# yuang-chen/of-spmm

Hardware: AMD Instinct MI355X
Metric: SpMM effective GFLOP/s + achieved HBM GB/s vs roofline, 1/2/4/8 MI355X (higher is better)
Workload: dtype f32; 1 GPU; products: CSR 2449029x2449029, 123718280 nnz x dense N=128; m=2449029, k=2449029, nnz=123718280, n=128, index=int32, parallelism=single GPU

## Files before the change

include/ofx_spmm.h:

```cpp
#ifndef OFX_SPMM_H_
#define OFX_SPMM_H_

#include <stddef.h>
#include <stdint.h>

#ifdef __cplusplus
extern "C" {
#endif

#define OFX_OK 0
#define OFX_EINVAL 1
#define OFX_EDEVICE 2
#define OFX_ENOMEM 3
#define OFX_EUNSUPPORTED 4
#define OFX_ECOMM 5
#define OFX_EWORKSPACE 6
#define OFX_EPLAN 7
#define OFX_EINTERNAL 8

#define OFX_DT_FLOAT 2
#define OFX_DT_DOUBLE 3
#define OFX_DT_INT32 5
#define OFX_DT_INT64 6
#define OFX_DT_FLOAT16 9
#define OFX_DT_BFLOAT16 11

const char* ofx_last_error(void);
const char* ofx_version(void);

int ofx_device_error_check(void);

#define OFX_DEBUG_PLAN_SPIN_LIMIT 1
#define OFX_DEBUG_THROW_IN_COMPUTE 2
#define OFX_DEBUG_EXCHANGE_STALL 3
int ofx_debug_set(int knob, int64_t value);

#define OFX_STRUCT_MAGIC 0x4F465831u

typedef struct ofx_spmm_options {
  uint32_t struct_size;
  uint32_t magic;
  int64_t split_threshold;
  int64_t chunk;
  int32_t ordered;
  int32_t variant;
  int64_t heavy_threshold;
  int32_t planned;
  int32_t reserved;
  int64_t range_nnz;
} ofx_spmm_options;
#define OFX_SPMM_OPTIONS_MIN_SIZE 48u
#define OFX_SPMM_OPTIONS_INIT \
  {(uint32_t)sizeof(ofx_spmm_options), OFX_STRUCT_MAGIC, 0, 0, 0, 0, 0, 0, 0, 0}

int64_t ofx_spmm_default_split(int64_t n);

int ofx_spmm_csr_workspace_size(int idx_dtype, int val_dtype, int64_t m, int64_t k, int64_t n,
                                int64_t nnz, const ofx_spmm_options* opts, size_t* bytes);

int ofx_spmm_csr(void* stream, int idx_dtype, int val_dtype, int64_t m, int64_t k, int64_t n,
                 int64_t nnz, const void* row_ptr, const void* col_idx, const void* values,
                 const void* b, int64_t ldb, void* c, int64_t ldc, int64_t row_begin,
                 int64_t row_end, void* workspace, size_t workspace_bytes,
                 const ofx_spmm_options* opts);

int ofx_spmm_csr_gathered(void* stream, int idx_dtype, int val_dtype, int64_t m, int64_t k,
                          int64_t n, int64_t nnz, const void* row_ptr, const void* col_idx,
                          const void* values, const void* values_perm, const void* b,
                          int64_t ldb, void* c, int64_t ldc, int64_t row_begin, int64_t row_end,
                          void* workspace, size_t workspace_bytes, const ofx_spmm_options* opts);

int ofx_spmm_csr_plan(void* stream, int idx_dtype, int val_dtype, int64_t m, int64_t k, int64_t n,
                      int64_t nnz, const void* row_ptr, int64_t row_begin, int64_t row_end,
                      void* workspace, size_t workspace_bytes, const ofx_spmm_options* opts);

int ofx_spmm_csr_describe(int idx_dtype, int val_dtype, int64_t m, int64_t k, int64_t n,
                          int64_t nnz, const void* b, int64_t ldb, const void* c, int64_t ldc,
                          int64_t row_begin, int64_t row_end, const ofx_spmm_options* opts,
                          char* buf, size_t buf_bytes);

int ofx_debug_bounds_read(uint64_t* out, int reset);

#define OFX_ACT_NONE 0
#define OFX_ACT_RELU 1
int ofx_spmm_csr_fused(void* stream, int idx_dtype, int val_dtype, int64_t m, int64_t k, int64_t n,
                       int64_t nnz, const void* row_ptr, const void* col_idx, const void* values,
                       const void* b, int64_t ldb, void* c, int64_t ldc, int64_t row_begin,
                       int64_t row_end, const void* bias, int activation, void* workspace,
                       size_t workspace_bytes, const ofx_spmm_options* opts);
int ofx_spmm_csr_fused_cpu(int num_threads, int idx_dtype, int val_dtype, int64_t m, int64_t k,
                           int64_t n, int64_t nnz, const void* row_ptr, const void* col_idx,
                           const void* values, const void* b, int64_t ldb, void* c, int64_t ldc,
                           int64_t row_begin, int64_t row_end, const void* bias, int activation,
                           const ofx_spmm_options* opts);

int ofx_csr_validate(void* stream, int idx_dtype, int64_t m, int64_t k, int64_t nnz,
                     const void* row_ptr, const void* col_idx, void* flag_dev);

int ofx_spmm_csr_cpu(int num_threads, int idx_dtype, int val_dtype, int64_t m, int64_t k,
                     int64_t n, int64_t nnz, const void* row_ptr, const void* col_idx,
                     const void* values, const void* b, int64_t ldb, void* c, int64_t ldc,
                     int64_t row_begin, int64_t row_end, const ofx_spmm_options* opts);

int ofx_csr_transpose_workspace_size(int idx_dtype, int64_t m, int64_t k, int64_t nnz,
                                     size_t* bytes);
int ofx_csr_transpose(void* stream, int idx_dtype, int64_t m, int64_t k, int64_t nnz,
                      const void* row_ptr, const void* col_idx, void* out_row_ptr,
// ... 151 lines not shown
                       void* d_bias, int relu, void* workspace, size_t workspace_bytes);
int ofx_relu_bias_grad_cpu(int num_threads, int val_dtype, int64_t m, int64_t n, const void* y,
                           int64_t ldy, const void* dy, int64_t lddy, void* dx, int64_t lddx,
                           void* d_bias, int relu);

int ofx_balanced_range(int64_t total, int64_t parts, int64_t idx, int64_t* begin, int64_t* end);
int ofx_csr_row_slice(void* stream, int idx_dtype, const void* row_ptr, int64_t row_begin,
                      int64_t row_end, void* out_row_ptr);
int ofx_csr_row_slice_host(int idx_dtype, const void* row_ptr, int64_t row_begin,
                           int64_t row_end, void* out_row_ptr, int64_t* nnz_begin,
                           int64_t* nnz_end);

int ofx_device_count(int* count);
int ofx_set_device(int device);
int ofx_get_device(int* device);
int ofx_device_synchronize(void);
int ofx_malloc(void** ptr, size_t bytes);
int ofx_free(void* ptr);
int ofx_host_malloc(void** ptr, size_t bytes);
int ofx_host_free(void* ptr);
int ofx_stream_create(void** stream);
int ofx_stream_destroy(void* stream);
int ofx_stream_sync(void* stream);
#define OFX_MEMCPY_H2D 1
#define OFX_MEMCPY_D2H 2
#define OFX_MEMCPY_D2D 3
#define OFX_MEMCPY_DEFAULT 4
int ofx_memcpy_async(void* stream, void* dst, const void* src, size_t bytes, int kind);
int ofx_memset_async(void* stream, void* dst, int value, size_t bytes);
int ofx_event_create(void** event, int timing);
int ofx_event_destroy(void* event);
int ofx_event_record(void* event, void* stream);
int ofx_event_sync(void* event);
int ofx_event_elapsed_ms(void* start, void* end, float* ms);
int ofx_stream_wait_event(void* stream, void* event);
int ofx_graph_exec_create(void** exec);
int ofx_graph_exec_destroy(void* exec);
int ofx_graph_exec_stats(void* exec, int* instantiated, int64_t* instantiations, int64_t* updates,
                         int64_t* launches);
int ofx_stream_begin_capture(void* stream);
int ofx_stream_is_capturing(void* stream, int* capturing);
int ofx_stream_end_capture(void* stream, void* exec);
int ofx_graph_launch(void* exec, void* stream);

#define OFX_UNIQUE_ID_BYTES 128
int ofx_comm_get_unique_id(void* uid_out );
int ofx_comm_init_rank(void** comm, int nranks, const void* uid, int rank);
int ofx_comm_init_rank_deadline(void** comm, int nranks, const void* uid, int rank,
                                double timeout_s);
int ofx_comm_set_timeouts(void* comm, double call_timeout_s, double device_timeout_s);
int ofx_comm_abort(void* comm);
int ofx_comm_destroy(void* comm);
int ofx_comm_count(void* comm, int* nranks, int* rank);
int ofx_allgather(void* stream, const void* in, void* out, size_t count, int dtype, void* comm);
int ofx_allgather_p2p(void* stream, void* buf, size_t count, int dtype, void* comm);
#define OFX_PEER_HANDLE_BYTES 96
#define OFX_PEER_MAX_RANKS 16
int ofx_peer_export(const void* ptr, void* handle_out);
int ofx_peer_open(const void* handle, void** ptr_out);
int ofx_peer_close(void* ptr);
int ofx_peer_publish(void* stream);
int ofx_peer_pull(void* stream, int nranks, int rank, const void* const* peer_bufs, void* buf,
                  uint64_t slot_bytes);
int ofx_peer_pull_host(int nranks, int rank, const void* const* peer_bufs, void* buf,
                       uint64_t slot_bytes);
int ofx_allgather_pull(void* stream, void* comm, const void* const* peer_bufs, void* buf,
// ... 45 lines not shown
                                  const ofx_tensor_desc* values, int64_t a_num_rows,
                                  int64_t a_num_cols, const ofx_tensor_desc* b,
                                  ofx_tensor_desc* out);
int ofx_functional_spmm_csr_tmp_size(const ofx_tensor_desc* row_ptr,
                                     const ofx_tensor_desc* col_idx,
                                     const ofx_tensor_desc* values, int64_t a_num_rows,
                                     int64_t a_num_cols, const ofx_tensor_desc* b,
                                     size_t* bytes);
int ofx_functional_spmm_csr(void* stream, const ofx_tensor_desc* row_ptr,
                            const ofx_tensor_desc* col_idx, const ofx_tensor_desc* values,
                            int64_t a_num_rows, int64_t a_num_cols, const ofx_tensor_desc* b,
                            ofx_tensor_desc* out, void* tmp, size_t tmp_bytes);
int ofx_functional_spmm_csr_global(void* stream, const ofx_tensor_desc* row_ptr,
                                   const ofx_tensor_desc* col_idx, const ofx_tensor_desc* values,
                                   int64_t a_num_rows, int64_t a_num_cols, const ofx_tensor_desc* b,
                                   int64_t b_logical_cols, ofx_tensor_desc* out, void* tmp,
                                   size_t tmp_bytes, int hierarchy_ndim, const int64_t* hierarchy,
                                   const int32_t* out_split_axes, int64_t parallel_id,
                                   int num_threads, size_t* tmp_size_out);
typedef struct ofx_spmm_attrs {
  uint32_t struct_size;
  uint32_t magic;
  int64_t static_csr;
} ofx_spmm_attrs;
#define OFX_SPMM_ATTRS_MIN_SIZE 16u
#define OFX_SPMM_ATTRS_INIT {(uint32_t)sizeof(ofx_spmm_attrs), OFX_STRUCT_MAGIC, 0}
int ofx_functional_spmm_csr_global_attrs(
    void* stream, const ofx_tensor_desc* row_ptr, const ofx_tensor_desc* col_idx,
    const ofx_tensor_desc* values, int64_t a_num_rows, int64_t a_num_cols,
    const ofx_tensor_desc* b, int64_t b_logical_cols, ofx_tensor_desc* out, void* tmp,
    size_t tmp_bytes, int hierarchy_ndim, const int64_t* hierarchy, const int32_t* out_split_axes,
    int64_t parallel_id, int num_threads, size_t* tmp_size_out, const ofx_spmm_attrs* attrs);
int ofx_spmm_static_plans(int64_t* entries, int64_t* plans, int64_t* hits, int release);

int ofx_functional_spmm_csr_ex(void* stream, const ofx_tensor_desc* row_ptr,
                               const ofx_tensor_desc* col_idx, const ofx_tensor_desc* values,
                               int64_t a_num_rows, int64_t a_num_cols, const ofx_tensor_desc* b,
                               ofx_tensor_desc* out, void* tmp, size_t tmp_bytes,
                               int64_t parallel_id, int64_t parallel_num, int out_split_axis,
                               int num_threads);
int ofx_functional_fused_spmm_csr(void* stream, const ofx_tensor_desc* row_ptr,
                                  const ofx_tensor_desc* col_idx, const ofx_tensor_desc* values,
                                  const ofx_tensor_desc* b, const ofx_tensor_desc* bias,
                                  int64_t a_num_rows, int64_t a_num_cols, int relu,
                                  ofx_tensor_desc* out, void* tmp, size_t tmp_bytes,
                                  size_t* tmp_size_out);
int ofx_functional_fused_spmm_csr_attrs(void* stream, const ofx_tensor_desc* row_ptr,
                                        const ofx_tensor_desc* col_idx,
                                        const ofx_tensor_desc* values, const ofx_tensor_desc* b,
                                        const ofx_tensor_desc* bias, int64_t a_num_rows,
                                        int64_t a_num_cols, int relu, ofx_tensor_desc* out,
                                        void* tmp, size_t tmp_bytes, size_t* tmp_size_out,
                                        const ofx_spmm_attrs* attrs);
int ofx_functional_sddmm_csr(void* stream, const ofx_tensor_desc* row_ptr,
                             const ofx_tensor_desc* col_idx, const ofx_tensor_desc* a,
                             const ofx_tensor_desc* b, int64_t a_num_rows, int64_t a_num_cols,
                             ofx_tensor_desc* out, void* tmp, size_t tmp_bytes,
                             size_t* tmp_size_out);
int ofx_functional_sddmm_csr_attrs(void* stream, const ofx_tensor_desc* row_ptr,
                                   const ofx_tensor_desc* col_idx, const ofx_tensor_desc* a,
                                   const ofx_tensor_desc* b, int64_t a_num_rows,
                                   int64_t a_num_cols, ofx_tensor_desc* out, void* tmp,
                                   size_t tmp_bytes, size_t* tmp_size_out,
                                   const ofx_spmm_attrs* attrs);
int ofx_functional_csr_transpose(void* stream, const ofx_tensor_desc* row_ptr,
                                 const ofx_tensor_desc* col_idx, int64_t a_num_rows,
// ... 118 lines not shown
```

of-spmm_amd/csrc/device_shim.cpp:

```cpp
#include <hip/hip_runtime.h>

#include <atomic>
#include <cstring>
#include <mutex>

#include "ofx_internal.h"

namespace {
constexpr int kErrWords = 16;
std::atomic<unsigned*> g_err_words{nullptr};
unsigned* g_err_dev = nullptr;
std::once_flag g_err_once;
}

namespace ofx {
unsigned* device_error_words() {
  std::call_once(g_err_once, [] {
    int count = 0;
    if (hipGetDeviceCount(&count) != hipSuccess || count <= 0) {
      (void)hipGetLastError();
      return;
    }
    hipStreamCaptureMode mode = hipStreamCaptureModeRelaxed;
    (void)hipThreadExchangeStreamCaptureMode(&mode);
// ... 64 lines not shown
extern "C" int ofx_device_synchronize(void) {
  return ::ofx::guarded(__func__, [&]() -> int {
    OFX_HIP_CHECK(hipDeviceSynchronize());
    OFX_TAKE_DEVICE_ERROR("device_synchronize");
    return OFX_OK;
  });
}
extern "C" int ofx_malloc(void** ptr, size_t bytes) {
  return ::ofx::guarded(__func__, [&]() -> int {
    OFX_REQUIRE(ptr, OFX_EINVAL, "malloc: NULL");
    *ptr = nullptr;
    if (bytes == 0) return OFX_OK;
    hipError_t e = hipMalloc(ptr, (bytes + 511) / 512 * 512);
    if (e != hipSuccess) {
      (void)hipGetLastError();
      return ofx::fail(OFX_ENOMEM, "hipMalloc(%zu) failed: %s", bytes, hipGetErrorString(e));
    }
    return OFX_OK;
  });
}
extern "C" int ofx_free(void* ptr) {
  return ::ofx::guarded(__func__, [&]() -> int {
    if (ptr) OFX_HIP_CHECK(hipFree(ptr));
    return OFX_OK;
  });
}
extern "C" int ofx_host_malloc(void** ptr, size_t bytes) {
  return ::ofx::guarded(__func__, [&]() -> int {
    OFX_REQUIRE(ptr, OFX_EINVAL, "host_malloc: NULL");
    OFX_HIP_CHECK(hipHostMalloc(ptr, bytes ? bytes : 1, hipHostMallocDefault));
    return OFX_OK;
  });
}
extern "C" int ofx_host_free(void* ptr) {
  return ::ofx::guarded(__func__, [&]() -> int {
    if (ptr) OFX_HIP_CHECK(hipHostFree(ptr));
    return OFX_OK;
  });
}
extern "C" int ofx_stream_create(void** stream) {
  return ::ofx::guarded(__func__, [&]() -> int {
    OFX_REQUIRE(stream, OFX_EINVAL, "stream_create: NULL");
    hipStream_t s;
    OFX_HIP_CHECK(hipStreamCreateWithFlags(&s, hipStreamNonBlocking));
    *stream = s;
    return OFX_OK;
  });
}
extern "C" int ofx_stream_destroy(void* stream) {
  return ::ofx::guarded(__func__, [&]() -> int {
    if (stream) OFX_HIP_CHECK(hipStreamDestroy(static_cast<hipStream_t>(stream)));
    return OFX_OK;
  });
}
extern "C" int ofx_stream_sync(void* stream) {
  return ::ofx::guarded(__func__, [&]() -> int {
    OFX_HIP_CHECK(hipStreamSynchronize(static_cast<hipStream_t>(stream)));
    OFX_TAKE_DEVICE_ERROR("stream_sync");
    return OFX_OK;
  });
}
extern "C" int ofx_memcpy_async(void* stream, void* dst, const void* src, size_t bytes, int kind) {
  return ::ofx::guarded(__func__, [&]() -> int {
    if (bytes == 0) return OFX_OK;
    hipMemcpyKind k;
    switch (kind) {
// ... 9 lines not shown
}
extern "C" int ofx_memset_async(void* stream, void* dst, int value, size_t bytes) {
  return ::ofx::guarded(__func__, [&]() -> int {
    if (bytes == 0) return OFX_OK;
    OFX_HIP_CHECK(hipMemsetAsync(dst, value, bytes, static_cast<hipStream_t>(stream)));
    return OFX_OK;
  });
}
extern "C" int ofx_event_create(void** event, int timing) {
  return ::ofx::guarded(__func__, [&]() -> int {
    OFX_REQUIRE(event, OFX_EINVAL, "event_create: NULL");
    hipEvent_t e;
    OFX_HIP_CHECK(hipEventCreateWithFlags(&e, timing ? hipEventDefault : hipEventDisableTiming));
    *event = e;
    return OFX_OK;
  });
}
extern "C" int ofx_event_destroy(void* event) {
  return ::ofx::guarded(__func__, [&]() -> int {
    if (event) OFX_HIP_CHECK(hipEventDestroy(static_cast<hipEvent_t>(event)));
    return OFX_OK;
  });
}
extern "C" int ofx_event_record(void* event, void* stream) {
  return ::ofx::guarded(__func__, [&]() -> int {
    OFX_HIP_CHECK(hipEventRecord(static_cast<hipEvent_t>(event), static_cast<hipStream_t>(stream)));
    return OFX_OK;
  });
}
extern "C" int ofx_event_sync(void* event) {
  return ::ofx::guarded(__func__, [&]() -> int {
    OFX_HIP_CHECK(hipEventSynchronize(static_cast<hipEvent_t>(event)));
    OFX_TAKE_DEVICE_ERROR("event_sync");
    return OFX_OK;
  });
}
extern "C" int ofx_event_elapsed_ms(void* start, void* end, float* ms) {
  return ::ofx::guarded(__func__, [&]() -> int {
    OFX_REQUIRE(ms, OFX_EINVAL, "event_elapsed_ms: NULL");
    OFX_HIP_CHECK(hipEventElapsedTime(ms, static_cast<hipEvent_t>(start),
                                      static_cast<hipEvent_t>(end)));
    return OFX_OK;
  });
}
extern "C" int ofx_stream_wait_event(void* stream, void* event) {
  return ::ofx::guarded(__func__, [&]() -> int {
    OFX_HIP_CHECK(hipStreamWaitEvent(static_cast<hipStream_t>(stream),
                                     static_cast<hipEvent_t>(event), 0));
    return OFX_OK;
  });
}

namespace {
struct GraphExec {
  hipGraphExec_t exec = nullptr;
  int device = -1;
  int64_t instantiations = 0;
  int64_t updates = 0;
  int64_t launches = 0;
};
}

extern "C" int ofx_graph_exec_create(void** exec) {
  return ::ofx::guarded(__func__, [&]() -> int {
    OFX_REQUIRE(exec, OFX_EINVAL, "graph_exec_create: NULL");
    *exec = new GraphExec();
// ... 109 lines not shown
```

of-spmm_amd/csrc/spmm_common.h:

```cpp
#ifndef OFX_SPMM_COMMON_H_
#define OFX_SPMM_COMMON_H_

#include <stdint.h>
#include <string.h>

#include "ofx_spmm.h"

#if defined(__HIPCC__) || defined(__HIP__)
#include <hip/hip_runtime.h>
#define OFX_HD __host__ __device__ __forceinline__
#else
#define OFX_HD static inline
#endif

namespace ofx {

struct bf16 {
  uint16_t x;
};
struct f16 {
  uint16_t x;
};

OFX_HD float bits_to_f32(uint32_t u) { return __builtin_bit_cast(float, u); }
// ... 89 lines not shown
  if (idx_dtype == OFX_DT_INT32) return f((int32_t*)nullptr);
  return f((int64_t*)nullptr);
}
template <typename F>
int by_types(int idx_dtype, int val_dtype, F&& f) {
  return by_index(idx_dtype, [&](auto* ip) -> int {
    switch (val_dtype) {
      case OFX_DT_FLOAT: return f((float*)nullptr, ip);
      case OFX_DT_DOUBLE: return f((double*)nullptr, ip);
      case OFX_DT_BFLOAT16: return f((bf16*)nullptr, ip);
      default: return f((f16*)nullptr, ip);
    }
  });
}

OFX_HD int64_t default_split(int64_t n) {
  int64_t t = n > 0 ? (int64_t)65536 / n : 512;
  if (t < 128) t = 128;
  if (t > 512) t = 512;
  int64_t p = 128;
  while (p * 2 <= t) p *= 2;
  return p;
}

struct Schedule {
  int64_t split;
  int64_t chunk;
  int64_t heavy;
  int32_t variant;
  int32_t planned;
  int32_t force_bin;
};

static inline Schedule resolve_schedule(int64_t n, const ofx_spmm_options* o) {
  Schedule s;
  s.variant = o ? o->variant : 0;
  s.planned = o ? o->planned : 0;
  s.force_bin = 0;
  const int64_t h = o ? o->heavy_threshold : 0;
  s.heavy = h > 0 ? h : (h < 0 ? INT64_MAX : 0);
  if (o && o->ordered) {
    s.split = INT64_MAX;
    s.chunk = INT64_MAX;
    return s;
  }
  s.split = (o && o->split_threshold > 0) ? o->split_threshold : default_split(n);
  s.chunk = (o && o->chunk > 0) ? o->chunk : s.split;
  if (s.chunk > s.split) s.chunk = s.split;
  return s;
}

OFX_HD int64_t auto_heavy(int64_t nrows, int64_t nnz) {
  const int64_t mean = nrows > 0 ? (nnz + nrows - 1) / nrows : 1;
  return 5 * mean < 16 ? 16 : 5 * mean;
}

OFX_HD int64_t num_chunks(int64_t len, int64_t chunk) { return len / chunk; }

OFX_HD uint64_t splitmix64(uint64_t x) {
  x += 0x9e3779b97f4a7c15ull;
  x = (x ^ (x >> 30)) * 0xbf58476d1ce4e5b9ull;
  x = (x ^ (x >> 27)) * 0x94d049bb133111ebull;
  return x ^ (x >> 31);
}
OFX_HD uint64_t hash2(uint64_t seed, uint64_t i) { return splitmix64(splitmix64(seed) ^ i); }
OFX_HD float u_pm1(uint64_t h) { return float((int64_t)(h >> 40) - (1 << 23)) * (1.0f / (1 << 23)); }
// ... 10 lines not shown
```

of-spmm_amd/csrc/spmm_csr.hip:

```cpp
#pragma clang fp contract(off)

#include <hip/hip_runtime.h>

#include <algorithm>
#include <climits>
#include <type_traits>

#include "ofx_internal.h"
#include "spmm_common.h"
#include "spmm_plan.h"
#include "spmm_launch.h"
#include "dbg_bounds.h"

namespace ofx {
namespace {

using plan::ws_layout;

template <typename I>
__global__ void csr_validate_kernel(const I* __restrict__ rp, const I* __restrict__ col,
                                    int64_t m, int64_t k, int64_t nnz, unsigned int* flag) {
  const int64_t stride = (int64_t)gridDim.x * blockDim.x;
  const int64_t t0 = (int64_t)blockIdx.x * blockDim.x + threadIdx.x;
  for (int64_t i = t0; i <= m; i += stride) {
// ... 132 lines not shown
    OFX_READ_OPTIONS(opts, "spmm_csr_describe");
    int rc = check_common(idx_dtype, val_dtype, m, k, n, nnz);
    if (rc) return rc;
    OFX_REQUIRE(0 <= row_begin && row_begin < row_end && row_end <= m && n > 0, OFX_EINVAL,
                "spmm_csr_describe: empty launch (rows [%lld, %lld), n=%lld)", (long long)row_begin,
                (long long)row_end, (long long)n);
    OFX_REQUIRE(ldb >= n && ldc >= n, OFX_EINVAL, "spmm_csr_describe: ldb / ldc < n");
    const int64_t nrows = row_end - row_begin;
    const int64_t nnz_est = launch_nnz(m, nrows, nnz, opts);
    Launch L{nullptr, nullptr, nullptr, nullptr, b, const_cast<void*>(c), ldb, ldc, row_begin, nrows,
             n, nnz, launch_schedule(nrows, nnz_est, n, resolve_schedule(n, opts)), nullptr, 0,
             nullptr, OFX_ACT_NONE, k, nullptr, nnz_est, buf, buf_bytes};
    if (idx_dtype == OFX_DT_INT32) return launch_idx<int32_t>(val_dtype, L);
    return launch_idx<int64_t>(val_dtype, L);
  });
}

extern "C" int ofx_spmm_csr_gathered(void* stream, int idx_dtype, int val_dtype, int64_t m,
                                     int64_t k, int64_t n, int64_t nnz, const void* row_ptr,
                                     const void* col_idx, const void* values,
                                     const void* values_perm, const void* b, int64_t ldb, void* c,
                                     int64_t ldc, int64_t row_begin, int64_t row_end,
                                     void* workspace, size_t workspace_bytes,
                                     const ofx_spmm_options* opts) {
  return ::ofx::guarded(__func__, [&]() -> int {
    OFX_REQUIRE(nnz == 0 || values_perm != nullptr, OFX_EINVAL,
                "spmm_csr_gathered: NULL values_perm with nnz=%lld", (long long)nnz);
    return spmm_entry(stream, idx_dtype, val_dtype, m, k, n, nnz, row_ptr, col_idx, values,
                      values_perm, b, ldb, c, ldc, row_begin, row_end, nullptr, OFX_ACT_NONE,
                      workspace, workspace_bytes, opts);
  });
}

extern "C" int ofx_spmm_csr_plan(void* stream, int idx_dtype, int val_dtype, int64_t m,
                                 int64_t k, int64_t n, int64_t nnz, const void* row_ptr,
                                 int64_t row_begin, int64_t row_end, void* workspace,
                                 size_t workspace_bytes, const ofx_spmm_options* opts) {
  return ::ofx::guarded(__func__, [&]() -> int {
    OFX_TAKE_DEVICE_ERROR("spmm_csr_plan");
    OFX_READ_OPTIONS(opts, "spmm_csr_plan");
    int rc = check_common(idx_dtype, val_dtype, m, k, n, nnz);
    if (rc) return rc;
    OFX_REQUIRE(0 <= row_begin && row_begin <= row_end && row_end <= m, OFX_EINVAL,
                "spmm_csr_plan: row range [%lld, %lld) outside [0, %lld)", (long long)row_begin,
                (long long)row_end, (long long)m);
    const int64_t nrows = row_end - row_begin;
    if (nrows == 0 || n == 0) return OFX_OK;
    const int64_t nnz_est = launch_nnz(m, nrows, nnz, opts);
    const Schedule s = launch_schedule(nrows, nnz_est, n, resolve_schedule(n, opts));
    if (use_small_form(nrows, nnz_est, n, s)) return OFX_OK;
    const plan::WsLayout w = plan::ws_layout(nrows, nnz, n, acc_bytes_of(val_dtype), s);
    if (w.total == 0) return OFX_OK;
    OFX_REQUIRE(row_ptr != nullptr, OFX_EINVAL, "spmm_csr_plan: NULL row_ptr");
    OFX_REQUIRE(workspace != nullptr && workspace_bytes >= w.total, OFX_EWORKSPACE,
                "spmm_csr_plan: workspace of %zu bytes is smaller than the %zu bytes required",
                workspace_bytes, w.total);
    hipStream_t st = static_cast<hipStream_t>(stream);
  #ifdef OFX_DEBUG_BOUNDS
    {
      dbg::HostBounds hb;
      hb.add(row_ptr, (uint64_t)((row_end + 1) * (idx_dtype == OFX_DT_INT32 ? 4 : 8)));
      hb.add(workspace, workspace_bytes);
      OFX_REQUIRE(hb.publish(st, 3ull << 48) == 0, OFX_EDEVICE, "spmm_csr_plan: debug bounds");
    }
  #endif
    plan::WorkList wl{};
    char* ws = static_cast<char*>(workspace);
    if (idx_dtype == OFX_DT_INT32)
      return plan::launch_plan<int32_t>(st, static_cast<const int32_t*>(row_ptr), row_begin, nrows,
                                        nnz_est, s, w, ws, &wl);
    return plan::launch_plan<int64_t>(st, static_cast<const int64_t*>(row_ptr), row_begin, nrows,
                                      nnz_est, s, w, ws, &wl);
  });
}

extern "C" int ofx_spmm_csr_fused(void* stream, int idx_dtype, int val_dtype, int64_t m,
                                  int64_t k, int64_t n, int64_t nnz, const void* row_ptr,
                                  const void* col_idx, const void* values, const void* b,
                                  int64_t ldb, void* c, int64_t ldc, int64_t row_begin,
                                  int64_t row_end, const void* bias, int activation,
                                  void* workspace, size_t workspace_bytes,
                                  const ofx_spmm_options* opts) {
  return ::ofx::guarded(__func__, [&]() -> int {
    return spmm_entry(stream, idx_dtype, val_dtype, m, k, n, nnz, row_ptr, col_idx, values, nullptr,
                      b, ldb, c, ldc, row_begin, row_end, bias, activation, workspace,
                      workspace_bytes, opts);
  });
}

extern "C" int ofx_csr_validate(void* stream, int idx_dtype, int64_t m, int64_t k, int64_t nnz,
                                const void* row_ptr, const void* col_idx, void* flag_dev) {
  return ::ofx::guarded(__func__, [&]() -> int {
    OFX_REQUIRE(is_index_dtype(idx_dtype), OFX_EUNSUPPORTED, "csr_validate: bad index dtype %d",
                idx_dtype);
    OFX_REQUIRE(row_ptr && flag_dev && (nnz == 0 || col_idx), OFX_EINVAL,
                "csr_validate: NULL pointer");
    hipStream_t s = static_cast<hipStream_t>(stream);
    OFX_HIP_CHECK(hipMemsetAsync(flag_dev, 0, sizeof(unsigned int), s));
    int64_t work = std::max<int64_t>(m + 1, nnz);
    int64_t grid = std::min<int64_t>((work + 255) / 256, 4096);
    if (grid < 1) grid = 1;
    if (idx_dtype == OFX_DT_INT32)
      hipLaunchKernelGGL(csr_validate_kernel<int32_t>, dim3((unsigned)grid), dim3(256), 0, s,
                         static_cast<const int32_t*>(row_ptr), static_cast<const int32_t*>(col_idx),
                         m, k, nnz, static_cast<unsigned int*>(flag_dev));
// ... 98 lines not shown
```

of-spmm_amd/csrc/spmm_csr_impl.h:

```cpp
#ifndef OFX_SPMM_CSR_IMPL_H_
#define OFX_SPMM_CSR_IMPL_H_
#pragma clang fp contract(off)

#include <hip/hip_runtime.h>

#include <algorithm>
#include <climits>
#include <cstdio>
#include <cstring>
#include <type_traits>

#include "ofx_internal.h"
#include "spmm_common.h"
#include "spmm_plan.h"
#include "spmm_launch.h"
#include "dbg_bounds.h"

namespace ofx {
namespace {


using plan::WorkList;
using plan::WsLayout;
using plan::launch_plan;
// ... 479 lines not shown
        for (int e = 0; e < VEC; ++e) lds[i * W + gl * VEC + e] = Num<T>::mul(vv[u], Num<T>::load(bv[u].v[e]));
      }
    }
    __builtin_amdgcn_fence(__ATOMIC_RELEASE, "wavefront");
    __builtin_amdgcn_wave_barrier();
    __builtin_amdgcn_fence(__ATOMIC_ACQUIRE, "wavefront");
    if (q == 0) {
#pragma unroll 8
      for (int i = 0; i < cnt; ++i)
#pragma unroll
        for (int e = 0; e < VEC; ++e) acc[e] = acc[e] + lds[i * W + gl * VEC + e];
    }
    __builtin_amdgcn_wave_barrier();
  }
}

template <typename T, int VEC, bool NT>
__device__ __forceinline__ void store_row(T* __restrict__ p, const typename Num<T>::acc (&acc)[VEC],
                                          const T* __restrict__ bias, int act) {
  if (!OFX_DOK(p, sizeof(Pack<T, VEC>)) || (bias && !OFX_DOK(bias, sizeof(T) * VEC))) return;
  Pack<T, VEC> o;
  if (bias == nullptr && act == OFX_ACT_NONE) {
#pragma unroll
    for (int e = 0; e < VEC; ++e) o.v[e] = Num<T>::store(acc[e]);
  } else {
#pragma unroll
    for (int e = 0; e < VEC; ++e) o.v[e] = epilogue<T>(acc[e], bias, e, act);
  }
  if constexpr (NT && (sizeof(o) == 16 || sizeof(o) == 8 || sizeof(o) == 4 || sizeof(o) == 2)) {
    using R = typename RawVec<sizeof(o)>::type;
    __builtin_nontemporal_store(__builtin_bit_cast(R, o), reinterpret_cast<R*>(p));
  } else {
    *reinterpret_cast<Pack<T, VEC>*>(p) = o;
  }
}

template <typename A, int VEC, bool COH = false>
__device__ __forceinline__ void store_partial(A* __restrict__ p, const A (&acc)[VEC]) {
  if constexpr (COH) {
#pragma unroll
    for (int e = 0; e < VEC; ++e) coh_store(p + e, acc[e]);
  } else {
    if (!OFX_DOK(p, sizeof(A) * VEC)) return;
#pragma unroll
    for (int e = 0; e < VEC; ++e) p[e] = acc[e];
  }
}

template <typename T, int VEC, int L, bool SH>
__device__ __forceinline__ void hub_tail(unsigned* __restrict__ arrive, int64_t slot0, int64_t nc,
                                         const typename Num<T>::acc* __restrict__ part,
                                         T* __restrict__ C, int64_t ldc, int64_t lr, int64_t n,
                                         int gl, bool member, int lead_lane,
                                         const T* __restrict__ bias, int act) {
#pragma clang fp contract(off)
  using A = typename Num<T>::acc;
  wait_stores();
  unsigned old = 0;
  if (member && gl == 0)
    old = __hip_atomic_fetch_add(arrive + slot0, 1u, __ATOMIC_RELAXED, __HIP_MEMORY_SCOPE_AGENT);
  old = __shfl(old, lead_lane);
  if ((int64_t)old != nc - 1) return;
  if (!member) return;
  for (int64_t c0 = 0; c0 < n; c0 += (int64_t)L * VEC) {
    int64_t cc = c0 + (int64_t)gl * VEC;
    if (cc >= n) continue;
// ... 327 lines not shown
      if (chain && active)
        store_row<T, VEC, K::NT>(C + hr * ldc + cc, split_row ? total : acc,
                                 bias ? bias + cc : nullptr, act);
    }
  }
}

#ifdef OFX_AB_WPE
#define OFX_MAIN_WPE __attribute__((amdgpu_waves_per_eu(OFX_AB_WPE)))
#else
#define OFX_MAIN_WPE
#endif
template <typename T>
__device__ __attribute__((noinline)) void poison_output(T* __restrict__ C, int64_t ldc,
                                                        int64_t nrows, int64_t n) {
  const T p = poison_value<T>();
  const int64_t total = nrows * n;
  const int64_t stride = (int64_t)gridDim.x * blockDim.x;
  for (int64_t e = (int64_t)blockIdx.x * blockDim.x + threadIdx.x; e < total; e += stride)
    C[(e / n) * ldc + e % n] = p;
}

template <typename T, typename I, typename K>
__global__ void __launch_bounds__(64 * K::WPB) OFX_MAIN_WPE
    spmm_main_kernel(const I* __restrict__ rp, const I* __restrict__ col,
                     const T* __restrict__ val, const I* __restrict__ vperm,
                     const T* __restrict__ B, int64_t ldb, int64_t kb,
                     T* __restrict__ C, int64_t ldc, int64_t row_begin, int64_t nrows, int64_t n,
                     int64_t split, int64_t chunk, int64_t heavy,
                     const unsigned long long* __restrict__ counters,
                     const int64_t* __restrict__ items, const int64_t* __restrict__ order,
                     typename Num<T>::acc* __restrict__ part, const T* __restrict__ bias,
                     int act, int64_t wave_blocks, int64_t block_base,
                     unsigned* __restrict__ arrive, unsigned* err) {
  using A = typename Num<T>::acc;
  constexpr int VEC = K::VEC, LPR = K::LPR, kWaves = K::WPB;
  const int64_t bid = block_base + (int64_t)blockIdx.x;
  if (counters != nullptr && !plan::plan_valid(counters)) {
    if (bid == 0 && threadIdx.x == 0) plan::raise_device_error(err, plan::kErrPlanInvalid);
    poison_output<T>(C, ldc, nrows, n);
    return;
  }
  constexpr int GPW = 64 / LPR;
  const int lane = threadIdx.x & 63;
  const int wave = __builtin_amdgcn_readfirstlane(threadIdx.x >> 6);
  const int gl = lane & (LPR - 1);
  const int gbase = lane & ~(LPR - 1);
  const int gsub = LPR == 64 ? 0 : lane / LPR;
  if constexpr (K::WH && LPR < 64) {
    using KW = WaveMap<K>;
    constexpr int WV = KW::VEC, WL = KW::LPR;
    if (bid < wave_blocks) {
      const int wgl = lane & (WL - 1);
      const int64_t nchunks = (int64_t)OFX_LD(counters + 0);
      const int64_t nheavy = (int64_t)OFX_LD(counters + 3) - (int64_t)OFX_LD(counters + 2);
      for (int64_t w = bid * kWaves + wave; w < nchunks + nheavy; w += wave_blocks * kWaves) {
        int64_t wr, wc = -1;
        if (w < nchunks) {
          wr = OFX_LD(items + (2 * w + 0));
          wc = OFX_LD(items + (2 * w + 1));
        } else {
          wr = plan::order_row(order, nrows, nheavy, w - nchunks);
        }
        wr = uniform64(wr);
        wc = uniform64(wc);
        const int64_t rs = (int64_t)OFX_LD(rp + (row_begin + wr));
        const int64_t re = (int64_t)OFX_LD(rp + (row_begin + wr + 1));
        int64_t j0 = rs, j1 = re;
        if (wc >= 0) {
          j0 = rs + wc * chunk;
          j1 = (re - j0 - chunk < chunk) ? re : j0 + chunk;
        }
        for (int64_t c0 = 0; c0 < n; c0 += (int64_t)WL * WV) {
          int64_t cc = c0 + (int64_t)wgl * WV;
          const bool active = cc < n;
          if constexpr (K::SH && WV > 1) {
            if (active && cc + WV > n) cc = n - WV;
          }
          A acc[WV];
#pragma unroll
          for (int e = 0; e < WV; ++e) acc[e] = A(0);
          if constexpr (K::XL) {
            __shared__ A xl_lds[K::WPB][KW::XL_FLOATS];
            accumulate_wave_xl<T, I, KW>(col, val, vperm, brows<T, K::BUF>(B, c0, cc, active, ldb, kb),
                                         j0, j1, lane, wgl, xl_lds[wave], acc);
          } else {
            accumulate_wave<T, I, KW>(col, val, vperm, brows<T, K::BUF>(B, c0, cc, active, ldb, kb),
                                      j0, j1, lane, wgl, acc);
          }
          if (active && lane < WL) {
            if (wc >= 0)
              store_partial<A, WV, K::LR>(part + w * n + cc, acc);
            else
              store_row<T, WV, K::NT>(C + wr * ldc + cc, acc, bias ? bias + cc : nullptr, act);
          }
        }
        if constexpr (K::LR) {
          if (wc >= 0)
            hub_tail<T, WV, WL, K::SH && (WV > 1)>(arrive, w - wc, num_chunks(re - rs, chunk), part, C, ldc,
                                       wr, n, wgl, lane < WL, 0, bias, act);
        }
      }
      return;
    }
  }
  if constexpr (K::BI) {
    if (bid < wave_blocks) {
      __shared__ __attribute__((aligned(16))) SmallLds<T, I, K> lds;
      constexpr int W = SmallForm<T, I, K>::W;
      const int64_t w = bid;
      const int64_t nchunks = (int64_t)OFX_LD(counters + 0);
      const int64_t nheavy = (int64_t)OFX_LD(counters + 3) - (int64_t)OFX_LD(counters + 2);
      if (w >= nchunks + nheavy) return;
      int64_t wr, wc = -1;
      if (w < nchunks) {
        wr = OFX_LD(items + (2 * w + 0));
        wc = OFX_LD(items + (2 * w + 1));
      } else {
        wr = plan::order_row(order, nrows, nheavy, w - nchunks);
      }
      wr = uniform64(wr);
      wc = uniform64(wc);
      const int64_t rs = (int64_t)OFX_LD(rp + (row_begin + wr));
      const int64_t re = (int64_t)OFX_LD(rp + (row_begin + wr + 1));
      int64_t j0 = rs, j1 = re;
      if (wc >= 0) {
        j0 = rs + wc * chunk;
        j1 = (re - j0 - chunk < chunk) ? re : j0 + chunk;
      }
      const int gb = wave * GPW + gsub;
      const bool chain = wave == 0 && gsub == 0;
      for (int64_t c0 = 0; c0 < n; c0 += W) {
        const int64_t cc = c0 + (int64_t)gl * VEC;
        const bool active = cc < n;
        A acc[VEC];
#pragma unroll
        for (int e = 0; e < VEC; ++e) acc[e] = A(0);
        block_accumulate<T, I, K>(col, val, vperm, brows<T, K::BUF>(B, c0, cc, active, ldb, kb), j0, j1, gb, gl,
                                  chain, lds, acc);
        if (chain && active) {
          if (wc >= 0)
            store_partial<A, VEC, K::LR>(part + w * n + cc, acc);
          else
            store_row<T, VEC, K::NT>(C + wr * ldc + cc, acc, bias ? bias + cc : nullptr, act);
        }
      }
      if constexpr (K::LR) {
        if (wc >= 0 && chain)
          hub_tail<T, VEC, LPR, K::SH>(arrive, w - wc, num_chunks(re - rs, chunk), part, C, ldc, wr,
                                       n, gl, true, gbase, bias, act);
      }
      return;
    }
  }
  int64_t g = ((bid - ((K::WH || K::BI) ? wave_blocks : 0)) * kWaves + wave) * GPW +
              gsub;
  if constexpr ((K::WH && LPR < 64) || K::BI) {
    if (order != nullptr)
      g += (int64_t)OFX_LD(counters + 0) + (int64_t)OFX_LD(counters + 3) -
           (int64_t)OFX_LD(counters + 2);
  }
  constexpr int64_t kIdxExcluded = 16;
#if defined(OFX_LIGHT_ORDER)
  constexpr bool kIdx = false;
#else
  constexpr bool kIdx = true;
#endif
  int64_t lr, c = -1;
  bool by_index = false;
  if (order == nullptr) {
    if (g >= nrows) return;
    lr = g;
  } else {
    const int64_t nchunks = (int64_t)OFX_LD(counters + 0);
    const int64_t nhubs = (int64_t)OFX_LD(counters + 1);
    const int64_t nheavy = (int64_t)OFX_LD(counters + 3) - (int64_t)OFX_LD(counters + 2);
#if defined(OFX_LIGHT_INDEX)
    const bool idx = true;
#else
    const bool idx = kIdx && (nhubs + nheavy) * kIdxExcluded <= nrows;
#endif
    if (g < nchunks) {
      lr = OFX_LD(items + (2 * g + 0));
      c = OFX_LD(items + (2 * g + 1));
    } else if (g < nchunks + nheavy || !idx) {
      const int64_t q = g - nchunks;
      if (q >= nrows - nhubs) return;
      lr = plan::order_row(order, nrows, nheavy, q);
    } else {
      lr = g - nchunks - nheavy;
      if (lr >= nrows) return;
      by_index = true;
    }
  }
  if constexpr (LPR == 64) {
    lr = uniform64(lr);
    c = uniform64(c);
  }
  const int64_t rs = (int64_t)OFX_LD(rp + (row_begin + lr));
  const int64_t re = (int64_t)OFX_LD(rp + (row_begin + lr + 1));
  if (by_index && (re - rs > split || re - rs > heavy)) return;
  int64_t j0 = rs, j1 = re;
  if (c >= 0) {
    j0 = rs + c * chunk;
    j1 = (re - j0 - chunk < chunk) ? re : j0 + chunk;
  }
  for (int64_t c0 = 0; c0 < n; c0 += (int64_t)LPR * VEC) {
    int64_t cc = c0 + (int64_t)gl * VEC;
    const bool active = cc < n;
    if constexpr (K::SH) {
      if (active && cc + VEC > n) cc = n - VEC;
    }
    A acc[VEC];
#pragma unroll
    for (int e = 0; e < VEC; ++e) acc[e] = A(0);
    accumulate<T, I, K>(col, val, vperm, brows<T, K::BUF>(B, c0, cc, active, ldb, kb), j0, j1, gl, gbase, active,
                        acc);
    if (active) {
      if (c >= 0)
        store_partial<A, VEC, K::LR>(part + g * n + cc, acc);
      else
        store_row<T, VEC, K::NT>(C + lr * ldc + cc, acc, bias ? bias + cc : nullptr, act);
    }
  }
  if constexpr (K::LR) {
    if (c >= 0)
      hub_tail<T, VEC, LPR, K::SH>(arrive, g - c, num_chunks(re - rs, chunk), part, C, ldc, lr, n,
                                   gl, true, gbase, bias, act);
  }
}


template <typename T, int VEC, int L>
__global__ void __launch_bounds__(kBlock)
    spmm_reduce_kernel(const unsigned long long* __restrict__ counters,
                       const int64_t* __restrict__ hubs,
                       const typename Num<T>::acc* __restrict__ part, T* __restrict__ C,
                       int64_t ldc, int64_t n, const T* __restrict__ bias, int act) {
#pragma clang fp contract(off)
  using A = typename Num<T>::acc;
  using P = Pack<A, VEC>;
  constexpr int kPre = 16;
  if (!plan::plan_valid(counters)) return;
  const int64_t nhubs = (int64_t)OFX_LD(counters + 1);
  const int gl = threadIdx.x % L;
  const int64_t groups = (int64_t)gridDim.x * (kBlock / L);
  for (int64_t h = (int64_t)blockIdx.x * (kBlock / L) + threadIdx.x / L; h < nhubs; h += groups) {
    const int64_t lr = OFX_LD(hubs + (3 * h + 0));
    const int64_t slot = OFX_LD(hubs + (3 * h + 1));
    const int64_t nc = OFX_LD(hubs + (3 * h + 2));
    for (int64_t c = (int64_t)gl * VEC; c < n; c += (int64_t)L * VEC) {
      const A* p = part + slot * n + c;
      A acc[VEC];
#pragma unroll
      for (int e = 0; e < VEC; ++e) acc[e] = A(0);
      int64_t q = 0;
      for (; q + kPre <= nc; q += kPre) {
        P v[kPre];
#pragma unroll
        for (int u = 0; u < kPre; ++u) v[u] = OFX_LD(reinterpret_cast<const P*>(p + (q + u) * n));
#pragma unroll
        for (int u = 0; u < kPre; ++u) {
#pragma unroll
          for (int e = 0; e < VEC; ++e) acc[e] = acc[e] + v[u].v[e];
        }
      }
      for (; q < nc; ++q) {
        const P v = OFX_LD(reinterpret_cast<const P*>(p + q * n));
#pragma unroll
        for (int e = 0; e < VEC; ++e) acc[e] = acc[e] + v.v[e];
      }
      if (bias && !OFX_DOK(bias + c, sizeof(T) * VEC)) continue;
#pragma unroll
      for (int e = 0; e < VEC; ++e) OFX_ST(&C[lr * ldc + c + e], epilogue<T>(acc[e], bias, c + e, act));
    }
  }
}

template <typename T, int VEC>
int launch_reduce_vec(hipStream_t s, int64_t max_hubs, int64_t n,
                      const unsigned long long* counters, const int64_t* hubs,
                      const typename Num<T>::acc* part, T* C, int64_t ldc, const T* bias, int act) {
  const int64_t lanes = (n + VEC - 1) / VEC;
  int l = 4;
  while (l < 64 && l < lanes) l *= 2;
  const int64_t per_block = kBlock / l;
  int64_t grid = (max_hubs + per_block - 1) / per_block;
  if (grid > kMaxReduceBlocks) grid = kMaxReduceBlocks;
#define OFX_REDUCE(LL)                                                                        \
  hipLaunchKernelGGL((spmm_reduce_kernel<T, VEC, LL>), dim3((unsigned)grid), dim3(kBlock), 0, s, \
                     counters, hubs, part, C, ldc, n, bias, act)
  switch (l) {
    case 4: OFX_REDUCE(4); break;
    case 8: OFX_REDUCE(8); break;
    case 16: OFX_REDUCE(16); break;
    case 32: OFX_REDUCE(32); break;
    default: OFX_REDUCE(64); break;
  }
#undef OFX_REDUCE
  OFX_HIP_CHECK(hipGetLastError());
  return OFX_OK;
}

template <typename T>
int launch_reduce(hipStream_t s, int64_t max_hubs, int64_t n, const unsigned long long* counters,
                  const int64_t* hubs, const typename Num<T>::acc* part, T* C, int64_t ldc,
                  const T* bias, int act) {
  using A = typename Num<T>::acc;
  constexpr int kVec = 16 / (int)sizeof(A);
  if ((n * (int64_t)sizeof(A)) % 16 == 0)
    return launch_reduce_vec<T, kVec>(s, max_hubs, n, counters, hubs, part, C, ldc, bias, act);
  return launch_reduce_vec<T, 1>(s, max_hubs, n, counters, hubs, part, C, ldc, bias, act);
}

int pick_vec(int elem_bytes, const Launch& L, int forced_vec, int cap = 16) {
  const int maxvec = std::min(16 / elem_bytes, cap);
  for (int v = maxvec; v >= 1; v /= 2) {
    if (forced_vec && v != forced_vec) continue;
    const size_t vb = (size_t)v * elem_bytes;
    if (L.n % v == 0 && L.ldb % v == 0 && L.ldc % v == 0 &&
        ((uintptr_t)L.b % vb) == 0 && ((uintptr_t)L.c % vb) == 0)
      return v;
  }
  return 0;
}

int pick_lpr(int64_t n, int vec) {
  const int64_t lanes = (n + vec - 1) / vec;
  int l = 4;
  while (l < 64 && l < lanes) l *= 2;
  return l;
}

template <typename T, typename I, typename K>
int describe_cfg(const Launch& L, const char* kind) {
  const char* form = std::strcmp(kind, "small") == 0 ? "small"
                     : K::BI                         ? "mid"
                     : (K::WH && K::HL > 0)          ? "narrow"
                     : K::PF                         ? "prefetch"
                                                     : "bandwidth";
  const size_t ws = std::strcmp(kind, "small") == 0
                        ? 0
                        : ws_layout(L.nrows, L.nnz, L.n, sizeof(typename Num<T>::acc), L.sched).total;
  std::snprintf(L.describe, L.describe_bytes,
                "form=%s kernel=%s VEC=%d LPR=%d U=%d WPB=%d NT=%d PF=%d WH=%d BI=%d BUF=%d SH=%d "
// ... 21 lines not shown
  void* zero = nullptr;
  OFX_HIP_CHECK(hipGetSymbolAddress(&zero, HIP_SYMBOL(g_zero_row)));
  hb.add(zero, kZeroRowBytes);
  const unsigned long long flags = (unsigned long long)K::NT | (unsigned long long)K::PF << 1 |
                                   (unsigned long long)K::BNT << 2 | (unsigned long long)K::WH << 3 |
                                   (unsigned long long)K::BI << 4 | (unsigned long long)K::BUF << 5 |
                                   (unsigned long long)K::SH << 6 | (unsigned long long)K::LR << 7;
  const unsigned long long tag = (unsigned long long)K::VEC | (unsigned long long)K::LPR << 8 |
                                 (unsigned long long)K::U << 16 | flags << 24 |
                                 (unsigned long long)K::HL << 32 | (unsigned long long)K::HU << 40 |
                                 kind << 48;
  OFX_REQUIRE(hb.publish(L.stream, tag) == 0, OFX_EDEVICE, "spmm_csr: debug bounds not published");
  return OFX_OK;
}
#endif

template <typename T, typename I, typename K>
int launch_cfg(const Launch& L) {
  if (L.describe != nullptr) return describe_cfg<T, I, K>(L, "main");
  using A = typename Num<T>::acc;
  constexpr int GPW = 64 / K::LPR;
  constexpr int64_t GPB = (int64_t)K::WPB * GPW;
  const I* rp = static_cast<const I*>(L.rp);
  const I* col = static_cast<const I*>(L.col);
  const T* val = static_cast<const T*>(L.val);
  const T* B = static_cast<const T*>(L.b);
  T* C = static_cast<T*>(L.c);
  const WsLayout w = ws_layout(L.nrows, L.nnz, L.n, sizeof(A), L.sched);
  const bool plan = w.total > 0;
#ifdef OFX_DEBUG_BOUNDS
  if (const int rc = debug_publish<T, I, K>(L, 1)) return rc;
#endif
  WorkList wl{};
  if (plan) {
    OFX_REQUIRE(L.ws != nullptr && L.ws_bytes >= w.total, OFX_EWORKSPACE,
                "spmm_csr: workspace of %zu bytes is smaller than the %zu bytes required",
                L.ws_bytes, w.total);
    if (L.sched.planned) {
      plan::worklist_of(w, static_cast<char*>(L.ws), &wl);
    } else {
      const int rc = launch_plan<I>(L.stream, rp, L.row_begin, L.nrows, L.nnz_est, L.sched, w,
                                    static_cast<char*>(L.ws), &wl);
      if (rc) return rc;
    }
  }
  unsigned long long* counters = wl.counters;
  int64_t *hub = wl.hubs, *items = wl.items, *order = wl.order;
  A* part = reinterpret_cast<A*>(wl.part);
  const int64_t heavy = L.sched.heavy == 0 ? auto_heavy(L.nrows, L.nnz_est) : L.sched.heavy;
  const int64_t heavy_bound =
      heavy == INT64_MAX ? 0 : std::min<int64_t>(L.nrows, L.nnz / (heavy + 1) + 1);
  const int64_t bi_items = w.max_chunks + heavy_bound;
  constexpr int64_t kWaveItemBlocks = 2048;
  const bool wh = K::WH && K::LPR < 64 && plan;
  const int64_t wave_blocks = wh ? std::min<int64_t>((bi_items + K::WPB - 1) / K::WPB, kWaveItemBlocks)
                              : (K::BI && plan) ? bi_items
                                                : 0;
  const int64_t work = L.nrows + (plan && !wh && !K::BI ? bi_items : 0);
  const int64_t grid = wave_blocks + (work + GPB - 1) / GPB;
  constexpr int64_t kLaunchBlocks = ((int64_t)1 << 31) / (64 * K::WPB);
  for (int64_t b0 = 0; b0 < grid; b0 += kLaunchBlocks) {
    const int64_t nb = std::min(kLaunchBlocks, grid - b0);
    hipLaunchKernelGGL((spmm_main_kernel<T, I, K>), dim3((unsigned)nb), dim3(64 * K::WPB), 0,
                       L.stream, rp, col, val, static_cast<const I*>(L.vperm), B, L.ldb, L.b_rows,
                       C, L.ldc, L.row_begin, L.nrows, L.n, plan ? L.sched.split : INT64_MAX,
                       plan ? L.sched.chunk : INT64_MAX, heavy, counters, items, order, part,
                       static_cast<const T*>(L.bias), L.act, wave_blocks, b0, wl.arrive,
                       plan ? device_error_words() : nullptr);
    OFX_HIP_CHECK(hipGetLastError());
  }
  if (plan && w.max_hubs > 0 && !K::LR)
    return launch_reduce<T>(L.stream, w.max_hubs, L.n, counters, hub, part, C, L.ldc,
                            static_cast<const T*>(L.bias), L.act);
  return OFX_OK;
}


template <typename T, typename I, typename K>
int launch_small(const Launch& L) {
  if (L.describe != nullptr) return describe_cfg<T, I, K>(L, "small");
  using SF = SmallForm<T, I, K>;
  const int64_t light =
      (L.sched.heavy > 0 && L.sched.heavy != INT64_MAX) ? L.sched.heavy : (int64_t)kSmallLight * K::U;
  const int64_t grid = (L.nrows + SF::RPB - 1) / SF::RPB;
#ifdef OFX_DEBUG_BOUNDS
  if (const int rc = debug_publish<T, I, K>(L, 2)) return rc;
#endif
  OFX_REQUIRE(grid < (int64_t)UINT32_MAX, OFX_EINVAL, "spmm_csr: too many rows (%lld)",
              (long long)L.nrows);
  hipLaunchKernelGGL((spmm_small_kernel<T, I, K>), dim3((unsigned)grid), dim3(64 * K::WPB), 0,
                     L.stream, static_cast<const I*>(L.rp), static_cast<const I*>(L.col),
                     static_cast<const T*>(L.val), static_cast<const I*>(L.vperm),
                     static_cast<const T*>(L.b), L.ldb, L.b_rows, static_cast<T*>(L.c), L.ldc,
                     L.row_begin,
                     L.nrows, L.n, L.sched.split, L.sched.chunk, light,
                     static_cast<const T*>(L.bias), L.act);
  OFX_HIP_CHECK(hipGetLastError());
  return OFX_OK;
}

template <typename T, typename I, typename K>
int launch_small_or_planned(const Launch& L) {
  if (use_small_form(L.nrows, L.nnz_est, L.n, L.sched)) return launch_small<T, I, K>(L);
  return launch_cfg<T, I, K>(L);
}

// ... 262 lines not shown
```

of-spmm_amd/csrc/spmm_plan.h:

```cpp
#ifndef OFX_SPMM_PLAN_H_
#define OFX_SPMM_PLAN_H_

#include <hip/hip_runtime.h>

#include <atomic>
#include <chrono>
#include <climits>

#include "ofx_internal.h"
#include "spmm_common.h"
#include "dbg_bounds.h"

namespace ofx {

template <typename A>
__device__ __forceinline__ A coh_load(const A* p) {
  if (!OFX_DOK(p, sizeof(A))) return A(0);
#ifdef OFX_AB_UNORDERED_HANDOFF
  return *(volatile const A*)p;
#else
  return __hip_atomic_load(const_cast<A*>(p), __ATOMIC_RELAXED, __HIP_MEMORY_SCOPE_AGENT);
#endif
}
template <typename A>
// ... 11 lines not shown
namespace {

constexpr int kBlock = 256;

inline size_t align_up(size_t x, size_t a) { return (x + a - 1) / a * a; }

constexpr int64_t kPlanRptRows = int64_t(1) << 18;
inline int plan_rpt(int64_t nrows) { return nrows <= kPlanRptRows ? 4 : 16; }
constexpr int kBins = 2;
constexpr int kPlanVals = 2 + kBins;
constexpr int64_t kOwnItems = 8;
constexpr int kLookWords = 16;
constexpr int kLookWin = 4;
constexpr unsigned long long kAgg = 1, kInc = 2;
constexpr int kEpoch = 4, kHostTag = 5, kOk = 6, kFail = 7, kPoison = 8, kCounterWords = 9;
constexpr int kSpinLimit = 1 << 22;

__host__ __device__ __forceinline__ unsigned long long plan_tag(unsigned long long epoch,
                                                               unsigned long long host_tag) {
  return (splitmix64(epoch * 0x9e3779b97f4a7c15ull + splitmix64(host_tag)) >> 2) | 1ull;
}

__device__ __forceinline__ bool plan_valid(const unsigned long long* __restrict__ counters) {
  const unsigned long long e = OFX_LDP(counters + kEpoch), h = OFX_LDP(counters + kHostTag);
  const unsigned long long ok = OFX_LDP(counters + kOk), fl = OFX_LDP(counters + kFail);
  const unsigned long long poison = OFX_LDP(counters + kPoison);
  return ok != 0 && ok == plan_tag(e - 1, h) && fl != ok && poison != ok;
}

constexpr int kErrPlanFailed = 0, kErrPlanInvalid = 1;
__device__ __forceinline__ void raise_device_error(unsigned* err, int which) {
  if (err != nullptr)
    __hip_atomic_store(err + which, 1u, __ATOMIC_RELAXED, __HIP_MEMORY_SCOPE_SYSTEM);
}

template <typename I>
__device__ __forceinline__ int plan_row(const I* __restrict__ rp, int64_t row_begin, int64_t nrows,
                                        int64_t g, int64_t split, int64_t chunk, int64_t heavy,
                                        int64_t& nc) {
  nc = 0;
  if (g >= nrows) return -2;
  const int64_t len = (int64_t)OFX_LDP(rp + (row_begin + g + 1)) -
                      (int64_t)OFX_LDP(rp + (row_begin + g));
  if (len > split) {
    nc = num_chunks(len, chunk);
    return -1;
  }
  if (heavy == INT64_MAX) return kBins - 1;
  int64_t t = heavy;
  for (int b = 0; b < kBins - 1; ++b, t >>= 2)
    if (len > t) return b;
  return kBins - 1;
}

__device__ __forceinline__ int64_t order_row(const int64_t* __restrict__ order, int64_t nrows,
                                             int64_t nheavy, int64_t q) {
  return q < nheavy ? OFX_LDP(order + (nrows - 1 - q)) : OFX_LDP(order + (q - nheavy));
}

__device__ __forceinline__ void block_scan_vals(int64_t (&v)[kPlanVals], int64_t (&tot)[kPlanVals]) {
  constexpr int kWaves = kBlock / 64;
  __shared__ int64_t wsum[kPlanVals][kWaves];
  const int lane = threadIdx.x & 63, wv = threadIdx.x >> 6;
  int64_t inc[kPlanVals];
#pragma unroll
  for (int i = 0; i < kPlanVals; ++i) inc[i] = v[i];
// ... 85 lines not shown
#pragma unroll
  for (int q = 0; q < RPT; ++q) {
    unsigned long long big = __ballot(cls[q] == -1 && nc[q] > kOwnItems);
    while (big) {
      const int src = __ffsll((long long)big) - 1;
      big &= big - 1;
      const int64_t g = (int64_t)__shfl((long long)(base + q), src);
      const int64_t s0 = (int64_t)__shfl((long long)first[q], src);
      const int64_t ncs = (int64_t)__shfl((long long)nc[q], src);
      for (int64_t c = threadIdx.x & 63; c < ncs; c += 64) {
        OFX_STP(items + (2 * (s0 + c) + 0), g);
        OFX_STP(items + (2 * (s0 + c) + 1), c);
      }
    }
  }
}

__device__ __forceinline__ unsigned long long look_status(unsigned long long* look, int64_t b) {
  return coh_load(look + b * kLookWords);
}
__device__ __forceinline__ void look_publish(unsigned long long* look, int64_t b,
                                             unsigned long long status) {
  wait_stores();
  coh_store(look + b * kLookWords, status);
}

template <int RPT, typename I>
__global__ void __launch_bounds__(kBlock)
    spmm_plan_kernel(const I* __restrict__ rp, int64_t row_begin, int64_t nrows, int64_t split,
                     int64_t chunk, int64_t heavy, unsigned long long* __restrict__ look,
                     unsigned long long host_tag, int64_t nblocks,
                     unsigned long long* __restrict__ counters, int64_t* __restrict__ hubs,
                     int64_t* __restrict__ items, int64_t* __restrict__ order,
                     unsigned* __restrict__ arrive, int spin_limit, unsigned* err) {
  __shared__ int64_t s_off[kPlanVals];
  __shared__ int s_fail;
  int cls[RPT];
  int64_t nc[RPT], v[kPlanVals], tot[kPlanVals];
  const int64_t b = blockIdx.x;
  const int64_t base = (b * kBlock + (int64_t)threadIdx.x) * RPT;
  const unsigned long long dev_epoch = threadIdx.x < 64 ? coh_load(counters + kEpoch) : 0ull;
  plan_thread<RPT>(rp, row_begin, nrows, base, split, chunk, heavy, cls, nc, v);
  block_scan_vals(v, tot);
  if (threadIdx.x < 64) {
    const unsigned long long epoch = plan_tag(dev_epoch, host_tag);
    const int lane = threadIdx.x;
    unsigned long long* my = look + b * kLookWords;
    if (lane == 0) {
#pragma unroll
      for (int i = 0; i < kPlanVals; ++i) {
        coh_store(my + 1 + i, (unsigned long long)tot[i]);
        if (b == 0) coh_store(my + 1 + kPlanVals + i, (unsigned long long)tot[i]);
      }
      look_publish(look, b, epoch << 2 | (b == 0 ? kInc : kAgg));
    }
    int64_t pre[kPlanVals] = {};
    bool failed = spin_limit == 0 && b > 0;
    for (int64_t end = failed ? 0 : b; end > 0; end -= 64 * kLookWin) {
      int64_t p[kLookWin];
      unsigned long long st[kLookWin];
#pragma unroll
      for (int w = 0; w < kLookWin; ++w) {
        p[w] = end - 1 - 64 * w - lane;
        st[w] = 0;
      }
      for (int spins = 0;;) {
        bool waiting = false;
// ... 44 lines not shown
      s_fail = failed ? 1 : 0;
      if (b > 0 && !failed) {
#pragma unroll
        for (int i = 0; i < kPlanVals; ++i)
          coh_store(my + 1 + kPlanVals + i, (unsigned long long)(pre[i] + tot[i]));
        look_publish(look, b, epoch << 2 | kInc);
      }
#pragma unroll
      for (int i = 0; i < kPlanVals; ++i) s_off[i] = pre[i];
    }
    if (lane == 0 && failed) {
      coh_store(counters + kFail, epoch);
      coh_store(counters + kPoison, plan_tag(dev_epoch + 1, host_tag));
      raise_device_error(err, kErrPlanFailed);
    }
    if (lane == 0 && b == nblocks - 1) {
      if (!failed) {
        OFX_STP(counters + 0, (unsigned long long)(pre[1] + tot[1]));
        OFX_STP(counters + 1, (unsigned long long)(pre[0] + tot[0]));
        OFX_STP(counters + 2, 0ull);
        OFX_STP(counters + 3, (unsigned long long)(pre[2] + tot[2]));
        OFX_STP(counters + kHostTag, host_tag);
      }
      OFX_STP(counters + kOk, failed ? 0ull : epoch);
      OFX_STP(counters + kEpoch, dev_epoch + 1);
    }
  }
  __syncthreads();
  if (s_fail) return;
  int64_t off[kPlanVals];
#pragma unroll
  for (int i = 0; i < kPlanVals; ++i) off[i] = s_off[i];
  plan_write_rows(cls, nc, v, off, base, nrows, hubs, items, order, arrive);
}

struct WsLayout {
  size_t counters, look, hubs, items, order, arrive, part, total;
  int64_t max_hubs, max_chunks, plan_blocks;
};

constexpr int64_t kMinBinRows = 16384;

WsLayout ws_layout(int64_t nrows, int64_t nnz, int64_t n, size_t acc_bytes, const Schedule& s) {
  WsLayout w{};
  const bool bin = s.heavy != INT64_MAX && (nrows >= kMinBinRows || s.force_bin);
  const bool hub = s.split != INT64_MAX && nnz > s.split;
  if (!bin && !hub) return w;
  w.max_hubs = s.split == INT64_MAX ? 0 : nnz / (s.split + 1) + 1;
  w.max_chunks = s.split == INT64_MAX ? 0 : nnz / s.chunk + 1;
  const int64_t rows_per_block = (int64_t)kBlock * plan_rpt(nrows);
  w.plan_blocks = (nrows + rows_per_block - 1) / rows_per_block;
  const int64_t look_blocks = (nrows + (int64_t)kBlock * 4 - 1) / ((int64_t)kBlock * 4);
  size_t off = 0;
  w.counters = off;
  off = align_up(off + kCounterWords * sizeof(unsigned long long), 256);
  w.look = off;
  off = align_up(off + (size_t)look_blocks * kLookWords * sizeof(unsigned long long), 256);
  w.hubs = off;
  off = align_up(off + (size_t)w.max_hubs * 3 * sizeof(int64_t), 256);
  w.items = off;
  off = align_up(off + (size_t)w.max_chunks * 2 * sizeof(int64_t), 256);
  w.order = off;
  off = align_up(off + (size_t)nrows * sizeof(int64_t), 256);
  w.arrive = off;
  off = align_up(off + (size_t)w.max_chunks * sizeof(unsigned), 256);
  w.part = off;
  off = align_up(off + (size_t)w.max_chunks * (size_t)n * acc_bytes, 256);
  w.total = off;
  return w;
}

struct WorkList {
  unsigned long long* counters;
  int64_t* hubs;
  int64_t* items;
  int64_t* order;
  unsigned* arrive;
  void* part;
};

inline void worklist_of(const WsLayout& w, char* ws, WorkList* wl) {
  wl->counters = reinterpret_cast<unsigned long long*>(ws + w.counters);
  wl->hubs = reinterpret_cast<int64_t*>(ws + w.hubs);
  wl->items = reinterpret_cast<int64_t*>(ws + w.items);
  wl->order = reinterpret_cast<int64_t*>(ws + w.order);
  wl->arrive = reinterpret_cast<unsigned*>(ws + w.arrive);
  wl->part = ws + w.part;
}

inline unsigned long long next_host_tag() {
  static std::atomic<unsigned long long> counter{
      splitmix64((unsigned long long)std::chrono::steady_clock::now().time_since_epoch().count() ^
                 (unsigned long long)(uintptr_t)&counter)};
  return (splitmix64(counter.fetch_add(1)) >> 2) | 1ull;
}

template <typename I>
int launch_plan(hipStream_t stream, const I* rp, int64_t row_begin, int64_t nrows, int64_t nnz,
                const Schedule& sched, const WsLayout& w, char* ws, WorkList* wl) {
  const int64_t heavy = sched.heavy == 0 ? auto_heavy(nrows, nnz) : sched.heavy;
  worklist_of(w, ws, wl);
  auto* look = reinterpret_cast<unsigned long long*>(ws + w.look);
  OFX_REQUIRE(w.plan_blocks < (int64_t)UINT32_MAX, OFX_EINVAL, "spmm_csr: too many rows to plan");
  const unsigned long long host_tag = next_host_tag();
  const int spin = debug_knob(OFX_DEBUG_PLAN_SPIN_LIMIT, kSpinLimit);
  unsigned* err = device_error_words();
  if (plan_rpt(nrows) == 4)
    hipLaunchKernelGGL((spmm_plan_kernel<4, I>), dim3((unsigned)w.plan_blocks), dim3(kBlock), 0,
                       stream, rp, row_begin, nrows, sched.split, sched.chunk, heavy, look, host_tag,
                       w.plan_blocks, wl->counters, wl->hubs, wl->items, wl->order, wl->arrive,
                       spin, err);
  else
    hipLaunchKernelGGL((spmm_plan_kernel<16, I>), dim3((unsigned)w.plan_blocks), dim3(kBlock), 0,
                       stream, rp, row_begin, nrows, sched.split, sched.chunk, heavy, look, host_tag,
                       w.plan_blocks, wl->counters, wl->hubs, wl->items, wl->order, wl->arrive,
                       spin, err);
  OFX_HIP_CHECK(hipGetLastError());
  return OFX_OK;
}

}
}
}

#endif
```

of-spmm_amd/oneflow/core/framework/framework.cpp:

```cpp
#include "oneflow/core/framework/framework.h"

#include "ofx_spmm.h"

#include <new>
#include <stdexcept>

#include "ofx_internal.h"

namespace oneflow {

void TestHookCompute(const char* op_name) {
  switch (ofx::debug_knob(OFX_DEBUG_THROW_IN_COMPUTE, 0)) {
    case 1: throw std::runtime_error(std::string(op_name) + ": injected by OFX_DEBUG_THROW_IN_COMPUTE");
    case 2: throw std::bad_alloc();
    case 3: throw 42;
    default: break;
  }
}

const char* DataType_Name(DataType dt) {
  switch (dt) {
    case kChar: return "kChar";
    case kFloat: return "kFloat";
    case kDouble: return "kDouble";
    case kInt8: return "kInt8";
    case kInt32: return "kInt32";
    case kInt64: return "kInt64";
    case kUInt8: return "kUInt8";
    case kFloat16: return "kFloat16";
    case kBFloat16: return "kBFloat16";
    case kBool: return "kBool";
    default: return "kInvalidDataType";
  }
}

const char* DeviceTypeName(DeviceType t) {
  switch (t) {
    case DeviceType::kCPU: return "cpu";
    case DeviceType::kCUDA: return "cuda";
    case DeviceType::kHIP: return "hip";
    case DeviceType::kMockDevice: return "mock";
    default: return "invalid";
  }
}

std::string Shape::ToString() const {
  std::ostringstream os;
  os << "(";
  for (size_t i = 0; i < dims_.size(); ++i) os << (i ? "," : "") << dims_[i];
  if (dims_.size() == 1) os << ",";
  os << ")";
// ... 135 lines not shown
```

of-spmm_amd/oneflow/core/framework/framework.h:

```cpp
#ifndef OFX_ONEFLOW_SHIM_FRAMEWORK_H_
#define OFX_ONEFLOW_SHIM_FRAMEWORK_H_

#include <cstdint>
#include <functional>
#include <map>
#include <memory>
#include <sstream>
#include <string>
#include <type_traits>
#include <utility>
#include <vector>

#include "ofx_spmm.h"

namespace oneflow {

enum DataType : int {
  kInvalidDataType = 0,
  kChar = 1,
  kFloat = 2,
  kDouble = 3,
  kInt8 = 4,
  kInt32 = 5,
  kInt64 = 6,
// ... 98 lines not shown

#define CHECK_OR_RETURN(cond) \
  if (!(cond)) return ::oneflow::ErrorBuilder(__FILE__, __LINE__, #cond)
#define OFX_CHECK_CMP_OR_RETURN_(a, b, op)                                                    \
  if (!((a)op(b)))                                                                            \
  return ::oneflow::ErrorBuilder(__FILE__, __LINE__, #a " " #op " " #b)                       \
         << "(" << (a) << " vs " << (b) << ") "
#define CHECK_EQ_OR_RETURN(a, b) OFX_CHECK_CMP_OR_RETURN_(a, b, ==)
#define CHECK_NE_OR_RETURN(a, b) OFX_CHECK_CMP_OR_RETURN_(a, b, !=)
#define CHECK_GE_OR_RETURN(a, b) OFX_CHECK_CMP_OR_RETURN_(a, b, >=)
#define CHECK_GT_OR_RETURN(a, b) OFX_CHECK_CMP_OR_RETURN_(a, b, >)
#define CHECK_LE_OR_RETURN(a, b) OFX_CHECK_CMP_OR_RETURN_(a, b, <=)
#define CHECK_LT_OR_RETURN(a, b) OFX_CHECK_CMP_OR_RETURN_(a, b, <)
#define CHECK_NOTNULL_OR_RETURN(p) CHECK_OR_RETURN((p) != nullptr)
#define JUST(expr)                                  \
  do {                                              \
    ::oneflow::Maybe<void> ofx_m_ = (expr);         \
    if (!ofx_m_.IsOk()) return ofx_m_;              \
  } while (0)

struct KernelCheckError {
  std::string msg;
};
#define OFX_KERNEL_CHECK(cond, msg)                                                          \
  do {                                                                                       \
    if (!(cond)) {                                                                           \
      std::ostringstream ofx_os_;                                                            \
      ofx_os_ << __FILE__ << ":" << __LINE__ << " CHECK failed: " #cond " " << msg;          \
      throw ::oneflow::KernelCheckError{ofx_os_.str()};                                      \
    }                                                                                        \
  } while (0)

void TestHookCompute(const char* op_name);

template <typename T>
struct GetDataType;
template <>
struct GetDataType<float> {
  static constexpr DataType value = kFloat;
};
template <>
struct GetDataType<double> {
  static constexpr DataType value = kDouble;
};
template <>
struct GetDataType<int32_t> {
  static constexpr DataType value = kInt32;
};
template <>
struct GetDataType<int64_t> {
  static constexpr DataType value = kInt64;
};

class BalancedSplitter {
 public:
  BalancedSplitter(int64_t total_num, int64_t split_num);
  std::pair<int64_t, int64_t> At(int64_t idx) const;

 private:
  int64_t total_, parts_;
};

class ParallelContext {
 public:
  ParallelContext(int64_t id = 0, int64_t num = 1) : id_(id), num_(num) {}
  int64_t parallel_id() const { return id_; }
// ... 591 lines not shown
```

of-spmm_amd/oneflow/core/functional/spmm_functor.cpp:

```cpp
#include <mutex>

#include "oneflow/core/framework/framework.h"
#include "oneflow/core/functional/spmm_functor.h"
#include "ofx_internal.h"
#include "ofx_spmm.h"

namespace oneflow {
namespace {

using DescMap = std::map<std::pair<std::string, int32_t>, user_op::TensorDesc>;

Shape ShapeOf(const ofx_tensor_desc* d) {
  std::vector<int64_t> dims;
  for (int i = 0; i < d->ndim; ++i) dims.push_back(d->shape[i]);
  return Shape(dims);
}

int ToStatus(const Maybe<void>& m) {
  if (m.IsOk()) return OFX_OK;
  return ofx::fail(OFX_EINVAL, "%s: %s", m.kind().c_str(), m.message().c_str());
}

Maybe<void> CheckDesc(const ofx_tensor_desc* d, const char* name) {
  const char* why = ofx::versioned_struct_problem(d, OFX_TENSOR_DESC_MIN_SIZE);
  CHECK_OR_RETURN(why == nullptr)
      << Error::RuntimeError() << name << ": ofx_tensor_desc " << why << " ("
      << OFX_TENSOR_DESC_MIN_SIZE << " bytes): initialise it with OFX_TENSOR_DESC_INIT";
  return Maybe<void>::Ok();
}

Maybe<void> CheckArgs(const ofx_tensor_desc* row_ptr, const ofx_tensor_desc* col_idx,
                      const ofx_tensor_desc* values, const ofx_tensor_desc* b) {
  CHECK_OR_RETURN(row_ptr && col_idx && values && b)
      << Error::RuntimeError() << "spmm_csr: NULL tensor argument";
  JUST(CheckDesc(row_ptr, "a_csr_row_ptr"));
  JUST(CheckDesc(col_idx, "a_csr_col_idx"));
// ... 158 lines not shown
  if (rc) return rc;
  const user_op::OpKernel* kernel = GetKernel(reg);

  user_op::Tensor t_rp(ShapeOf(row_ptr), (DataType)row_ptr->dtype, row_ptr->data);
  user_op::Tensor t_ci(ShapeOf(col_idx), (DataType)col_idx->dtype, col_idx->data);
  user_op::Tensor t_v(ShapeOf(values), (DataType)values->dtype, values->data);
  user_op::Tensor t_b(ShapeOf(b), (DataType)b->dtype, b->data, b->ndim == 2 ? b->stride[0] : -1);
  user_op::Tensor t_o(ShapeOf(out), (DataType)out->dtype, out->data, out->stride[0]);
  user_op::Tensor t_tmp(Shape({(int64_t)tmp_bytes}), kChar, tmp);
  std::map<std::pair<std::string, int32_t>, user_op::Tensor*> tensors = {
      {{"a_csr_row_ptr", 0}, &t_rp}, {{"a_csr_col_idx", 0}, &t_ci}, {{"a_csr_values", 0}, &t_v},
      {{"b", 0}, &t_b},              {{"out", 0}, &t_o}};
  if (tmp) tensors[{"tmp_buffer", 0}] = &t_tmp;
  const DeviceType dev = b->device < 0 ? DeviceType::kCPU : DeviceType::kHIP;
  ep::CpuStream cpu_stream(num_threads);
  ep::HipStream hip_stream(stream, b->device);
  ep::Stream* s = dev == DeviceType::kCPU ? static_cast<ep::Stream*>(&cpu_stream)
                                          : static_cast<ep::Stream*>(&hip_stream);
  user_op::AttrMap attrs;
  if (const user_op::OpRegistryResult* op =
          user_op::UserOpRegistryMgr::Get().GetOpRegistryResult("spmm_csr"))
    for (const auto& a : op->attrs) attrs[a.first] = a.second;
  attrs["a_num_rows"] = m;
  attrs["a_num_cols"] = k;
  attrs["static_csr"] = static_csr;
  user_op::OpKernelState* kstate = nullptr;
  if (state != nullptr) {
    if (!*state) {
      user_op::KernelInitContext ictx(ParallelContext(pl.parallel_id, pl.parallel_num()),
                                      ParallelDesc(pl.hierarchy), dev, "compiled_job");
      *state = kernel->CreateOpKernelState(&ictx);
    }
    kstate = state->get();
  } else if (static_csr != 0) {
    kstate = EagerKernelState(reg, kernel, b->device, dev);
  }
  user_op::KernelCacheContext cache_ctx(ParallelContext(pl.parallel_id, pl.parallel_num()),
                                        ParallelDesc(pl.hierarchy),
                                        {{"out", pl.out_sbp}, {"b", pl.b_sbp}},
                                        {{"out", logical_od}}, dev);
  user_op::KernelComputeContext ctx(s, tensors, attrs, dev);
  try {
    std::shared_ptr<user_op::OpKernelCache> cache = kernel->InitOpKernelCache(&cache_ctx);
    if (phys_rows == 0 || od.shape().At(1) == 0) {
      if (!kernel->AlwaysComputeWhenAllOutputsEmpty()) return OFX_OK;
    }
    kernel->Compute(&ctx, kstate, cache.get());
  } catch (const KernelCheckError& e) {
    return ofx::fail(OFX_EINVAL, "%s", e.msg.c_str());
  }
  return OFX_OK;
}

}

int SpmmCsrGlobalWithState(void* stream, const ofx_tensor_desc* row_ptr,
                           const ofx_tensor_desc* col_idx, const ofx_tensor_desc* values,
                           int64_t m, int64_t k, const ofx_tensor_desc* b, int64_t b_logical_cols,
                           ofx_tensor_desc* out, void* tmp, size_t tmp_bytes, int hierarchy_ndim,
                           const int64_t* hierarchy, const int32_t* out_split_axes,
                           int64_t parallel_id, int64_t static_csr,
                           std::shared_ptr<user_op::OpKernelState>* state) {
  Placement pl;
  int rc = ToStatus(MakePlacement(hierarchy_ndim, hierarchy, out_split_axes, parallel_id, &pl));
  if (rc) return rc;
  return RunSpmmCsr(stream, row_ptr, col_idx, values, m, k, b, b_logical_cols, out, tmp,
                    tmp_bytes, pl, 0, nullptr, static_csr, state);
// ... 55 lines not shown
extern "C" int ofx_functional_spmm_csr_global_attrs(
    void* stream, const ofx_tensor_desc* row_ptr, const ofx_tensor_desc* col_idx,
    const ofx_tensor_desc* values, int64_t a_num_rows, int64_t a_num_cols,
    const ofx_tensor_desc* b, int64_t b_logical_cols, ofx_tensor_desc* out, void* tmp,
    size_t tmp_bytes, int hierarchy_ndim, const int64_t* hierarchy, const int32_t* out_split_axes,
    int64_t parallel_id, int num_threads, size_t* tmp_size_out, const ofx_spmm_attrs* attrs) {
  return ::ofx::guarded(__func__, [&]() -> int {
    int64_t static_csr = 0;
    if (attrs != nullptr) {
      const char* why = ofx::versioned_struct_problem(attrs, OFX_SPMM_ATTRS_MIN_SIZE);
      OFX_REQUIRE(why == nullptr, OFX_EINVAL,
                  "spmm_csr: ofx_spmm_attrs %s (%u bytes): initialise it with OFX_SPMM_ATTRS_INIT",
                  why ? why : "", OFX_SPMM_ATTRS_MIN_SIZE);
      static_csr = attrs->static_csr;
    }
    Placement pl;
    int rc = ToStatus(MakePlacement(hierarchy_ndim, hierarchy, out_split_axes, parallel_id, &pl));
    if (rc) return rc;
    return RunSpmmCsr(stream, row_ptr, col_idx, values, a_num_rows, a_num_cols, b, b_logical_cols,
                      out, tmp, tmp_bytes, pl, num_threads, tmp_size_out, static_csr);
  });
}

extern "C" int ofx_spmm_static_plans(int64_t* entries, int64_t* plans, int64_t* hits,
                                     int release) {
  return ::ofx::guarded(__func__, [&]() -> int {
    int64_t e = 0, p = 0, h = 0;
    std::lock_guard<std::mutex> lock(g_eager_states_mu);
    for (auto& kv : g_eager_states)
      if (kv.second) SpmmCsrPlanStateStats(kv.second.get(), &e, &p, &h, release != 0);
    if (entries) *entries = e;
    if (plans) *plans = p;
    if (hits) *hits = h;
    return OFX_OK;
  });
}

extern "C" int ofx_functional_spmm_csr_ex(void* stream, const ofx_tensor_desc* row_ptr,
                                          const ofx_tensor_desc* col_idx,
                                          const ofx_tensor_desc* values, int64_t a_num_rows,
                                          int64_t a_num_cols, const ofx_tensor_desc* b,
                                          ofx_tensor_desc* out, void* tmp, size_t tmp_bytes,
                                          int64_t parallel_id, int64_t parallel_num,
                                          int out_split_axis, int num_threads) {
  return ::ofx::guarded(__func__, [&]() -> int {
    OFX_REQUIRE(out_split_axis != 1 || parallel_num == 1, OFX_EINVAL,
                "spmm_csr_ex: a column split needs the logical width: use "
                "ofx_functional_spmm_csr_global");
    const int64_t h = parallel_num;
    const int32_t ax = out_split_axis;
    return ofx_functional_spmm_csr_global(stream, row_ptr, col_idx, values, a_num_rows, a_num_cols,
                                          b, -1, out, tmp, tmp_bytes, 1, &h, &ax, parallel_id,
                                          num_threads, nullptr);
  });
}

extern "C" int ofx_functional_spmm_csr(void* stream, const ofx_tensor_desc* row_ptr,
                                       const ofx_tensor_desc* col_idx,
                                       const ofx_tensor_desc* values, int64_t a_num_rows,
                                       int64_t a_num_cols, const ofx_tensor_desc* b,
                                       ofx_tensor_desc* out, void* tmp, size_t tmp_bytes) {
  return ::ofx::guarded(__func__, [&]() -> int {
    return RunSpmmCsr(stream, row_ptr, col_idx, values, a_num_rows, a_num_cols, b, -1, out, tmp,
                      tmp_bytes, Placement(), 0, nullptr);
  });
}
// ... 117 lines not shown
    sc.logical = logical;
    *tmp_size_out = reg->infer_tmp_size ? reg->infer_tmp_size(&sc) : 0;
    return Maybe<void>::Ok();
  }
  std::vector<std::unique_ptr<user_op::Tensor>> hold;
  std::map<std::pair<std::string, int32_t>, user_op::Tensor*> tensors;
  auto add = [&](const Arg& a) {
    hold.emplace_back(new user_op::Tensor(ShapeOf(a.d), (DataType)a.d->dtype, a.d->data,
                                          a.d->ndim == 2 ? a.d->stride[0] : -1));
    tensors[{a.name, 0}] = hold.back().get();
  };
  for (const Arg& a : ins) add(a);
  for (const Arg& o : outs) {
    CHECK_OR_RETURN(o.d != nullptr) << Error::RuntimeError() << op_name << ": NULL output " << o.name;
    JUST(CheckDesc(o.d, o.name));
    const user_op::TensorDesc& want = ictx.OutputTensorDesc(o.name, 0);
    CHECK_OR_RETURN(ShapeOf(o.d) == want.shape() && (DataType)o.d->dtype == want.data_type() &&
                    o.d->device == device)
        << Error::RuntimeError() << op_name << ": output " << o.name << " must be "
        << want.shape().ToString() << " of dtype " << DataType_Name(want.data_type());
    JUST(CheckUnitColumnStride(o.d, o.name));
    add(o);
  }
  user_op::Tensor t_tmp(Shape({(int64_t)tmp_bytes}), kChar, tmp);
  if (tmp) tensors[{"tmp_buffer", 0}] = &t_tmp;
  ep::CpuStream cpu_stream(num_threads);
  ep::HipStream hip_stream(stream, device);
  ep::Stream* s = device < 0 ? static_cast<ep::Stream*>(&cpu_stream) : static_cast<ep::Stream*>(&hip_stream);
  user_op::KernelComputeContext ctx(s, tensors, attrs, rc.device_type());
  const user_op::OpKernel* kernel = GetKernel(reg);
  std::shared_ptr<user_op::OpKernelCache> cache;
  auto sc = attrs.find("static_csr");
  user_op::OpKernelState* kstate = nullptr;
  if (sc != attrs.end() && static_cast<int64_t>(sc->second) != 0)
    kstate = EagerKernelState(reg, kernel, device, rc.device_type());
  try {
    if (pl != nullptr) {
      user_op::KernelCacheContext cache_ctx(ParallelContext(pl->parallel_id, pl->parallel_num()),
                                            ParallelDesc(pl->hierarchy), nd_sbp, logical,
                                            rc.device_type());
      cache = kernel->InitOpKernelCache(&cache_ctx);
    }
    kernel->Compute(&ctx, kstate, cache.get());
  } catch (const KernelCheckError& e) {
    return Maybe<void>("KernelCheckError", e.msg);
  }
  return Maybe<void>::Ok();
}

}
}

extern "C" int ofx_functional_sddmm_csr(void* stream, const ofx_tensor_desc* row_ptr,
                                        const ofx_tensor_desc* col_idx, const ofx_tensor_desc* a,
                                        const ofx_tensor_desc* b, int64_t a_num_rows,
                                        int64_t a_num_cols, ofx_tensor_desc* out, void* tmp,
                                        size_t tmp_bytes, size_t* tmp_size_out) {
  return ofx_functional_sddmm_csr_attrs(stream, row_ptr, col_idx, a, b, a_num_rows, a_num_cols,
                                        out, tmp, tmp_bytes, tmp_size_out, nullptr);
}

extern "C" int ofx_functional_sddmm_csr_attrs(void* stream, const ofx_tensor_desc* row_ptr,
                                              const ofx_tensor_desc* col_idx,
                                              const ofx_tensor_desc* a, const ofx_tensor_desc* b,
                                              int64_t a_num_rows, int64_t a_num_cols,
                                              ofx_tensor_desc* out, void* tmp, size_t tmp_bytes,
                                              size_t* tmp_size_out, const ofx_spmm_attrs* attrs) {
// ... 294 lines not shown
```

of-spmm_amd/oneflow/core/functional/spmm_functor.h:

```cpp
#ifndef OFX_ONEFLOW_CORE_FUNCTIONAL_SPMM_FUNCTOR_H_
#define OFX_ONEFLOW_CORE_FUNCTIONAL_SPMM_FUNCTOR_H_

#include <memory>

#include "oneflow/core/framework/framework.h"
#include "ofx_spmm.h"

namespace oneflow {

int SpmmCsrGlobalWithState(void* stream, const ofx_tensor_desc* row_ptr,
                           const ofx_tensor_desc* col_idx, const ofx_tensor_desc* values,
                           int64_t m, int64_t k, const ofx_tensor_desc* b, int64_t b_logical_cols,
                           ofx_tensor_desc* out, void* tmp, size_t tmp_bytes, int hierarchy_ndim,
                           const int64_t* hierarchy, const int32_t* out_split_axes,
                           int64_t parallel_id, int64_t static_csr,
                           std::shared_ptr<user_op::OpKernelState>* state);

bool SpmmCsrPlanStateStats(user_op::OpKernelState* state, int64_t* entries, int64_t* plans,
                           int64_t* hits, bool release);

int EdgeSoftmaxCsr(void* stream, const ofx_tensor_desc* row_ptr, const ofx_tensor_desc* col_idx,
                   const ofx_tensor_desc* in, const ofx_tensor_desc* grad, ofx_tensor_desc* out,
                   void* tmp, size_t tmp_bytes, size_t* tmp_size_out, int num_threads);

int EdgeSoftmaxCsrHeads(void* stream, const ofx_tensor_desc* row_ptr,
                        const ofx_tensor_desc* col_idx, const ofx_tensor_desc* in,
                        const ofx_tensor_desc* grad, ofx_tensor_desc* out, void* tmp,
                        size_t tmp_bytes, size_t* tmp_size_out, int num_threads);

}

#endif
```

of-spmm_amd/oneflow/user/kernels/spmm_kernel.cpp:

```cpp
#include "oneflow/core/framework/framework.h"
#include "oneflow/core/functional/spmm_functor.h"
#include "oneflow/user/kernels/spmm_plan_state.h"
#include "ofx_spmm.h"

namespace oneflow {

bool SpmmCsrPlanStateStats(user_op::OpKernelState* state, int64_t* entries, int64_t* plans,
                           int64_t* hits, bool release) {
  auto* s = dynamic_cast<SpmmCsrPlanState*>(state);
  if (s == nullptr) return false;
  if (release) s->Release();
  s->Stats(entries, plans, hits);
  return true;
}

namespace {

class SpmmCsrOpKernelCache final : public user_op::OpKernelCache {
 public:
  SpmmCsrOpKernelCache(int64_t lower, int64_t upper, int64_t logical_n)
      : lower_(lower), upper_(upper), logical_n_(logical_n) {}
  ~SpmmCsrOpKernelCache() override = default;
  int64_t lower() const { return lower_; }
  int64_t upper() const { return upper_; }
  int64_t logical_n() const { return logical_n_; }

 private:
  const int64_t lower_;
  const int64_t upper_;
  const int64_t logical_n_;
};

std::shared_ptr<user_op::OpKernelCache> CreateSpmmCsrOpKernelCache(user_op::KernelCacheContext* ctx) {
  const user_op::TensorDesc* out_logical = ctx->LogicalTensorDesc4ArgNameAndIndex("out", 0);
  const Shape& shape = out_logical->shape();
  int64_t lower = 0, upper = shape.At(0);
  if (ctx->parallel_ctx().parallel_num() > 1) {
    const TensorSliceView view =
        GetTensorSliceView4ParallelId(*ctx->parallel_desc().hierarchy(),
                                      ctx->NdSbp4ArgNameAndIndex("out", 0), shape,
                                      ctx->parallel_ctx().parallel_id());
    lower = view.At(0).begin();
    upper = view.At(0).end();
  }
  return std::make_shared<SpmmCsrOpKernelCache>(lower, upper, shape.At(1));
}

ofx_spmm_options OptionsOf(const SpmmCsrOpKernelCache* cache) {
  ofx_spmm_options o = OFX_SPMM_OPTIONS_INIT;
  if (cache != nullptr) o.split_threshold = ofx_spmm_default_split(cache->logical_n());
  return o;
}

int DtCode(DataType dt) { return static_cast<int>(dt); }

void UseStaticSpmmPlan(SpmmCsrPlanState* plans, int64_t static_csr, ep::HipStream* hs,
                       const void* row_ptr, int idx_dt, int val_dt, int64_t m, int64_t k,
                       int64_t n, int64_t nnz, int64_t row_begin, int64_t row_end,
                       const char* op_name, ofx_spmm_options* opts, void** ws, size_t* ws_bytes,
                       StaticPlan* sp) {
  if (row_end <= row_begin || n <= 0) return;
  size_t need = 0;
  const int rc = ofx_spmm_csr_workspace_size(idx_dt, val_dt, m, k, n, nnz, opts, &need);
  OFX_KERNEL_CHECK(rc == OFX_OK, op_name << " workspace query failed: " << ofx_last_error());
  void* stream = hs->hip_stream();
  const SpmmCsrPlanState::Key key{static_csr, row_ptr, plans->key_on_stream() ? stream : nullptr,
                                  hs->device_index(), idx_dt, val_dt, m, k, n, nnz, row_begin,
                                  row_end, opts->split_threshold, opts->chunk,
                                  opts->heavy_threshold, opts->range_nnz};
  auto plan = [&](void* sws, size_t bytes) {
    return ofx_spmm_csr_plan(stream, idx_dt, val_dt, m, k, n, nnz, row_ptr, row_begin, row_end,
                             sws, bytes, opts);
  };
  if (UseStaticPlan(plans, key, need, hs->IsGraphCapturing(), op_name, plan, ws, ws_bytes, sp))
    opts->planned = 1;
}

template <DeviceType device_type>
void ComputeSpmmCsr(user_op::KernelComputeContext* ctx, const user_op::OpKernelCache* cache,
                    const user_op::Tensor* bias, bool relu, const char* op_name,
                    SpmmCsrPlanState* plans = nullptr, int64_t static_csr = 0) {
  TestHookCompute(op_name);
  const user_op::Tensor* row_ptr = ctx->Tensor4ArgNameAndIndex("a_csr_row_ptr", 0);
  const user_op::Tensor* col_idx = ctx->Tensor4ArgNameAndIndex("a_csr_col_idx", 0);
  const user_op::Tensor* values = ctx->Tensor4ArgNameAndIndex("a_csr_values", 0);
  const user_op::Tensor* b = ctx->Tensor4ArgNameAndIndex("b", 0);
  user_op::Tensor* out = ctx->Tensor4ArgNameAndIndex("out", 0);
  const int64_t m = ctx->Attr<int64_t>("a_num_rows");
  const int64_t k = ctx->Attr<int64_t>("a_num_cols");
  OFX_KERNEL_CHECK(b->shape_view().NumAxes() == 2, "b Numdims should be equal to 2. ");
  OFX_KERNEL_CHECK(out->shape_view().NumAxes() == 2, "out Numdims should be equal to 2. ");
  OFX_KERNEL_CHECK(out->data_type() == b->data_type(), "out datatype should be equal to b. ");
  const int64_t n = out->shape_view().At(1);
  const int64_t nnz = col_idx->shape_view().elem_cnt();
  int64_t row_begin = 0;
  int64_t row_end = m;
  const auto* range = dynamic_cast<const SpmmCsrOpKernelCache*>(cache);
  OFX_KERNEL_CHECK(cache == nullptr || range != nullptr, "unexpected kernel cache type");
  if (range != nullptr) {
    row_begin = range->lower();
    row_end = range->upper();
  }
  ofx_spmm_options opts = OptionsOf(range);
  OFX_KERNEL_CHECK(out->shape_view().At(0) == row_end - row_begin,
                   "out rows " << out->shape_view().At(0) << " != row range "
                               << row_end - row_begin);
  if (bias != nullptr)
    OFX_KERNEL_CHECK(bias->shape_view().elem_cnt() == n && bias->data_type() == b->data_type(),
                     "bias must be [" << n << "] of b's dtype");
  const int idx_dt = DtCode(row_ptr->data_type());
  const int val_dt = DtCode(values->data_type());
  const void* bias_ptr = bias ? bias->dptr() : nullptr;
  const int act = relu ? OFX_ACT_RELU : OFX_ACT_NONE;
  int rc;
  if (device_type == DeviceType::kHIP) {
    user_op::Tensor* tmp = ctx->Tensor4ArgNameAndIndex("tmp_buffer", 0);
    void* ws = tmp ? tmp->mut_dptr() : nullptr;
    size_t ws_bytes = tmp ? (size_t)tmp->shape_view().elem_cnt() : 0;
    ep::HipStream* hs = ctx->stream()->As<ep::HipStream>();
    void* stream = hs->hip_stream();
    StaticPlan sp;
    if (plans != nullptr && static_csr != 0)
      UseStaticSpmmPlan(plans, static_csr, hs, row_ptr->dptr(), idx_dt, val_dt, m, k, n, nnz,
                        row_begin, row_end, op_name, &opts, &ws, &ws_bytes, &sp);
    rc = ofx_spmm_csr_fused(stream, idx_dt, val_dt, m, k, n, nnz, row_ptr->dptr(),
                            col_idx->dptr(), values->dptr(), b->dptr(), b->row_stride(),
                            out->mut_dptr(), out->row_stride(), row_begin, row_end, bias_ptr, act,
                            ws, ws_bytes, &opts);
    if (rc != OFX_OK && sp.keyed) plans->Drop(sp.key, hs->IsGraphCapturing());
  } else {
    const int threads = ctx->stream()->As<ep::CpuStream>()->num_threads();
    rc = ofx_spmm_csr_fused_cpu(threads, idx_dt, val_dt, m, k, n, nnz, row_ptr->dptr(),
                                col_idx->dptr(), values->dptr(), b->dptr(), b->row_stride(),
                                out->mut_dptr(), out->row_stride(), row_begin, row_end, bias_ptr,
                                act, &opts);
  }
  OFX_KERNEL_CHECK(rc == OFX_OK, op_name << " kernel failed (" << rc << "): " << ofx_last_error());
}

template <DeviceType device_type>
class SpmmCsrKernel final : public user_op::OpKernel, public user_op::CudaGraphSupport {
 public:
  SpmmCsrKernel() = default;
  ~SpmmCsrKernel() override = default;

  std::shared_ptr<user_op::OpKernelCache> InitOpKernelCache(
      user_op::KernelCacheContext* ctx) const override {
    return CreateSpmmCsrOpKernelCache(ctx);
  }

  std::shared_ptr<user_op::OpKernelState> CreateOpKernelState(
      user_op::KernelInitContext* ctx) const override {
    if (device_type != DeviceType::kHIP) return nullptr;
    return std::make_shared<SpmmCsrPlanState>(!ctx->has_stream_name_hint());
  }

  bool AlwaysComputeWhenAllOutputsEmpty() const override { return false; }

 private:
  using user_op::OpKernel::Compute;
  void Compute(user_op::KernelComputeContext* ctx, user_op::OpKernelState* state,
               const user_op::OpKernelCache* cache) const override {
// ... 93 lines not shown
                          row_begin, row_end, "spmm_csr_gathered", &opts, &ws, &ws_bytes, &sp);
      rc = ofx_spmm_csr_gathered(hs->hip_stream(), idx_dt, val_dt, m, k, n, nnz, row_ptr->dptr(),
                                 col_idx->dptr(), values->dptr(), perm->dptr(), b->dptr(),
                                 b->row_stride(), out->mut_dptr(), out->row_stride(), row_begin,
                                 row_end, ws, ws_bytes, &opts);
      if (rc != OFX_OK && sp.keyed) plans->Drop(sp.key, hs->IsGraphCapturing());
    } else {
      const size_t vbytes = (size_t)nnz * (size_t)GetSizeOfDataType(values->data_type());
      OFX_KERNEL_CHECK(nnz == 0 || ws_bytes >= vbytes, "tmp buffer smaller than the values");
      rc = ofx_gather_values_host(idx_dt, val_dt, nnz, perm->dptr(), values->dptr(), ws);
      if (rc == OFX_OK)
        rc = ofx_spmm_csr_cpu(ctx->stream()->As<ep::CpuStream>()->num_threads(), idx_dt, val_dt,
                              m, k, n, nnz, row_ptr->dptr(), col_idx->dptr(), ws, b->dptr(),
                              b->row_stride(), out->mut_dptr(), out->row_stride(), row_begin,
                              row_end, &opts);
    }
    OFX_KERNEL_CHECK(rc == OFX_OK,
                     "spmm_csr_gathered kernel failed (" << rc << "): " << ofx_last_error());
  }
};

size_t InferSpmmCsrGatheredCpuTmpSize(user_op::InferSizeContext* ctx) {
  const user_op::TensorDesc& values = ctx->InputTensorDesc("a_csr_values", 0);
  return (size_t)values.shape().elem_cnt() * (size_t)GetSizeOfDataType(values.data_type());
}

size_t InferSpmmCsrTmpSize(user_op::InferSizeContext* ctx) {
  const user_op::TensorDesc& row_ptr = ctx->InputTensorDesc("a_csr_row_ptr", 0);
  const user_op::TensorDesc& col_idx = ctx->InputTensorDesc("a_csr_col_idx", 0);
  const user_op::TensorDesc& b = ctx->InputTensorDesc("b", 0);
  const user_op::TensorDesc* out_logical = ctx->LogicalTensorDesc4ArgNameAndIndex("out", 0);
  ofx_spmm_options o = OFX_SPMM_OPTIONS_INIT;
  if (out_logical != nullptr) o.split_threshold = ofx_spmm_default_split(out_logical->shape().At(1));
  size_t bytes = 0;
  const int rc = ofx_spmm_csr_workspace_size(
      DtCode(row_ptr.data_type()), DtCode(b.data_type()), ctx->Attr<int64_t>("a_num_rows"),
      ctx->Attr<int64_t>("a_num_cols"), b.shape().At(1), col_idx.shape().At(0), &o, &bytes);
  return rc == OFX_OK ? bytes : 0;
}

}

#define REGISTER_SPMM_CSR_KERNEL_OF(op, kernel, device, dtype, itype)                          \
  REGISTER_USER_KERNEL(op)                                                                    \
      .SetCreateFn<kernel<device>>()                                                          \
      .SetIsMatchedHob((user_op::HobDeviceType() == device)                                   \
                       && (user_op::HobDataType("out", 0) == dtype)                           \
                       && (user_op::HobDataType("a_csr_row_ptr", 0) == itype))                \
      .SetInferTmpSizeFn(device == DeviceType::kHIP                                           \
                             ? std::function<size_t(user_op::InferSizeContext*)>(             \
                                   InferSpmmCsrTmpSize)                                       \
                             : std::function<size_t(user_op::InferSizeContext*)>(             \
                                   [](user_op::InferSizeContext*) -> size_t { return 0; }));

#define REGISTER_SPMM_CSR_KERNEL(device, dtype, itype)                                     \
  REGISTER_SPMM_CSR_KERNEL_OF("spmm_csr", SpmmCsrKernel, device, dtype, itype)            \
  REGISTER_SPMM_CSR_KERNEL_OF("fused_spmm_csr", FusedSpmmCsrKernel, device, dtype, itype)

#define REGISTER_SPMM_CSR_KERNEL_ALL_INDEX(device, dtype) \
  REGISTER_SPMM_CSR_KERNEL(device, dtype, kInt32)         \
  REGISTER_SPMM_CSR_KERNEL(device, dtype, kInt64)

#define REGISTER_SPMM_CSR_KERNEL_ALL(device)              \
  REGISTER_SPMM_CSR_KERNEL_ALL_INDEX(device, kFloat)      \
  REGISTER_SPMM_CSR_KERNEL_ALL_INDEX(device, kDouble)     \
  REGISTER_SPMM_CSR_KERNEL_ALL_INDEX(device, kFloat16)    \
// ... 29 lines not shown
```

of-spmm_amd/oneflow/user/kernels/spmm_plan_state.h:

```cpp
#ifndef OFX_ONEFLOW_USER_KERNELS_SPMM_PLAN_STATE_H_
#define OFX_ONEFLOW_USER_KERNELS_SPMM_PLAN_STATE_H_

#include <list>
#include <mutex>

#include "oneflow/core/framework/framework.h"
#include "ofx_spmm.h"

namespace oneflow {

class SpmmCsrPlanState final : public user_op::OpKernelState {
 public:
  struct Key {
    int64_t static_csr;
    const void* row_ptr;
    const void* stream;
    int device, idx_dt, val_dt;
    int64_t m, k, n, nnz, row_begin, row_end, split, chunk, heavy, range_nnz;
    bool operator==(const Key& o) const {
      return static_csr == o.static_csr && row_ptr == o.row_ptr && stream == o.stream &&
             device == o.device && idx_dt == o.idx_dt && val_dt == o.val_dt && m == o.m &&
             k == o.k && n == o.n && nnz == o.nnz && row_begin == o.row_begin &&
             row_end == o.row_end && split == o.split && chunk == o.chunk && heavy == o.heavy &&
             range_nnz == o.range_nnz;
    }
  };
  static constexpr size_t kMaxPlans = 8;

  explicit SpmmCsrPlanState(bool key_on_stream) : key_on_stream_(key_on_stream) {}
  ~SpmmCsrPlanState() override { Release(); }
  bool key_on_stream() const { return key_on_stream_; }
  std::recursive_mutex& launch_mutex() { return mu_; }

  int Acquire(const Key& key, size_t bytes, bool capturing, void** ws, bool* planned) {
    std::lock_guard<std::recursive_mutex> lock(mu_);
    *ws = nullptr;
    *planned = false;
    for (auto it = entries_.begin(); it != entries_.end(); ++it) {
      if (it->key == key && it->bytes >= bytes) {
        entries_.splice(entries_.begin(), entries_, it);
        if (capturing) it->pinned = true;
        *ws = it->ws;
        *planned = true;
        ++hits_;
        return OFX_OK;
      }
    }
    if (capturing) return OFX_OK;
    int rc = OFX_OK;
    if (entries_.size() >= kMaxPlans) {
      auto victim = entries_.end();
      for (auto it = entries_.begin(); it != entries_.end(); ++it)
        if (!it->pinned) victim = it;
      if (victim != entries_.end()) {
        rc = WithDevice(victim->key.device, [&]() {
          const int r = ofx_device_synchronize();
          return r != OFX_OK ? r : ofx_free(victim->ws);
        });
        entries_.erase(victim);
        if (rc != OFX_OK) return rc;
// ... 5 lines not shown
    entries_.push_front(Entry{key, p, bytes, false});
    *ws = p;
    ++plans_;
    return OFX_OK;
  }

  void Drop(const Key& key, bool capturing) {
    std::lock_guard<std::recursive_mutex> lock(mu_);
    for (auto it = entries_.begin(); it != entries_.end(); ++it) {
      if (it->key == key) {
        if (capturing || it->pinned) {
          retired_.push_back(*it);
        } else {
          WithDevice(it->key.device, [&]() {
            ofx_device_synchronize();
            return ofx_free(it->ws);
          });
        }
        entries_.erase(it);
        return;
      }
    }
  }

  void Stats(int64_t* entries, int64_t* plans, int64_t* hits) {
    std::lock_guard<std::recursive_mutex> lock(mu_);
    *entries += (int64_t)entries_.size();
    *plans += plans_;
    *hits += hits_;
  }

  void Release() {
    std::lock_guard<std::recursive_mutex> lock(mu_);
    for (auto* list : {&retired_, &entries_}) {
      for (Entry& e : *list) {
        WithDevice(e.key.device, [&]() {
          ofx_device_synchronize();
          return ofx_free(e.ws);
        });
      }
      list->clear();
    }
  }

 private:
  struct Entry {
    Key key;
    void* ws;
    size_t bytes;
    bool pinned;
  };
  template <typename F>
  static int WithDevice(int device, F&& f) {
    int prev = -1;
    if (ofx_get_device(&prev) != OFX_OK) prev = -1;
    if (prev != device && ofx_set_device(device) != OFX_OK) return OFX_EDEVICE;
    const int rc = f();
    if (prev >= 0 && prev != device) ofx_set_device(prev);
    return rc;
  }

  const bool key_on_stream_;
  std::recursive_mutex mu_;
  std::list<Entry> entries_;
  std::list<Entry> retired_;
  int64_t plans_ = 0, hits_ = 0;
};

struct StaticPlan {
  SpmmCsrPlanState::Key key{};
  bool keyed = false;
  std::unique_lock<std::recursive_mutex> hold;
};

template <typename PlanFn>
bool UseStaticPlan(SpmmCsrPlanState* plans, const SpmmCsrPlanState::Key& key, size_t need,
                   bool capturing, const char* op_name, PlanFn&& plan_fn, void** ws,
                   size_t* ws_bytes, StaticPlan* sp) {
  if (need == 0) return false;
  sp->hold = std::unique_lock<std::recursive_mutex>(plans->launch_mutex());
  sp->key = key;
  void* sws = nullptr;
  bool planned = false;
  int rc = plans->Acquire(key, need, capturing, &sws, &planned);
  OFX_KERNEL_CHECK(rc == OFX_OK, op_name << " static_csr plan workspace: " << ofx_last_error());
  if (sws == nullptr) return false;
  sp->keyed = true;
  if (!planned) {
    rc = plan_fn(sws, need);
    if (rc != OFX_OK) plans->Drop(key, capturing);
    OFX_KERNEL_CHECK(rc == OFX_OK, op_name << " kernel failed (" << rc << "): " << ofx_last_error());
  }
  *ws = sws;
  *ws_bytes = need;
  return true;
}

}

// ... 2 lines not shown
```

of-spmm_amd/oneflow_spmm/_C.py:

```python
from __future__ import annotations

import ctypes

import torch

from . import _lib
from ._lib import LIB, TensorDesc, check

_TORCH_TO_DT = {
    torch.float32: _lib.DT_FLOAT,
    torch.float64: _lib.DT_DOUBLE,
    torch.float16: _lib.DT_FLOAT16,
    torch.bfloat16: _lib.DT_BFLOAT16,
    torch.int32: _lib.DT_INT32,
    torch.int64: _lib.DT_INT64,
}
_DT_TO_TORCH = {v: k for k, v in _TORCH_TO_DT.items()}


def dtype_code(dt: torch.dtype) -> int:
    try:
        return _TORCH_TO_DT[dt]
    except KeyError:
        raise TypeError(f"spmm_csr: unsupported dtype {dt}") from None
# ... 91 lines not shown
    else:
        check(LIB.ofx_functional_spmm_csr_global(None, *common, None, None, 0, *tail,
                                                 ctypes.byref(tmp_bytes)), "spmm_csr")
    tmp = None
    if tmp_bytes.value:
        tmp = torch.empty(tmp_bytes.value, dtype=torch.uint8, device=bb.device)
    if static_csr:
        attrs = _lib.SpmmAttrs()
        attrs.static_csr = int(static_csr)
        check(LIB.ofx_functional_spmm_csr_global_attrs(
            current_stream_handle(bb), *common, ctypes.byref(d_o),
            tmp.data_ptr() if tmp is not None else None, tmp_bytes.value, *tail, None,
            ctypes.byref(attrs)), "spmm_csr")
    else:
        check(LIB.ofx_functional_spmm_csr_global(current_stream_handle(bb), *common,
                                                 ctypes.byref(d_o),
                                                 tmp.data_ptr() if tmp is not None else None,
                                                 tmp_bytes.value, *tail, None), "spmm_csr")
    if memo is None and len(_SIG_MEMO) < 4096:
        _SIG_MEMO[key] = (tuple(out.shape), out.dtype, tmp_bytes.value)
    return out


_SIG_MEMO: dict = {}


def static_plans(release: bool = False) -> dict:
    e, p, h = ctypes.c_int64(), ctypes.c_int64(), ctypes.c_int64()
    check(LIB.ofx_spmm_static_plans(ctypes.byref(e), ctypes.byref(p), ctypes.byref(h),
                                    1 if release else 0), "spmm_static_plans")
    return {"entries": e.value, "plans": p.value, "hits": h.value}


def fused_spmm_csr(a_csr_row_ptr: torch.Tensor, a_csr_col_idx: torch.Tensor,
                   a_csr_values: torch.Tensor, a_num_rows: int, a_num_cols: int, b: torch.Tensor,
                   bias: torch.Tensor | None = None, *, relu: bool = False,
                   out: torch.Tensor | None = None, static_csr: int = 0) -> torch.Tensor:
    rp = _prep(a_csr_row_ptr, "a_csr_row_ptr")
    ci = _prep(a_csr_col_idx, "a_csr_col_idx")
    vals = _prep(a_csr_values, "a_csr_values")
    bb = _prep(b, "b", matrix=True)
    bs = _prep(bias, "bias") if bias is not None else None
    d_rp, d_ci, d_v, d_b = desc(rp), desc(ci), desc(vals), desc(bb)
    d_bias = ctypes.byref(desc(bs)) if bs is not None else None
    od = TensorDesc()
    check(LIB.ofx_functional_spmm_csr_infer(ctypes.byref(d_rp), ctypes.byref(d_ci), ctypes.byref(d_v),
                                            int(a_num_rows), int(a_num_cols), ctypes.byref(d_b),
                                            ctypes.byref(od)), "fused_spmm_csr")
    if out is None:
        out = torch.empty((od.shape[0], od.shape[1]), dtype=_DT_TO_TORCH[od.dtype], device=bb.device)
    d_o = desc(out)
    args = (ctypes.byref(d_rp), ctypes.byref(d_ci), ctypes.byref(d_v), ctypes.byref(d_b), d_bias,
            int(a_num_rows), int(a_num_cols), 1 if relu else 0, ctypes.byref(d_o))
    size = ctypes.c_size_t(0)
    check(LIB.ofx_functional_fused_spmm_csr(None, *args, None, 0, ctypes.byref(size)), "fused_spmm_csr")
    tmp = None
    if size.value and bb.device.type != "cpu":
        tmp = torch.empty(size.value, dtype=torch.uint8, device=bb.device)
    attrs = None
    if static_csr:
        attrs = _lib.SpmmAttrs()
        attrs.static_csr = int(static_csr)
        attrs = ctypes.byref(attrs)
    check(LIB.ofx_functional_fused_spmm_csr_attrs(current_stream_handle(bb), *args,
                                                  tmp.data_ptr() if tmp is not None else None,
                                                  size.value if tmp is not None else 0, None,
# ... 352 lines not shown
```

of-spmm_amd/oneflow_spmm/_lib.py:

```python
from __future__ import annotations

import ctypes
import os

_HERE = os.path.dirname(os.path.abspath(__file__))
LIB_PATH = os.environ.get("OFX_SPMM_LIB") or os.path.join(_HERE, "libofx_spmm.so")

DT_FLOAT, DT_DOUBLE, DT_INT32, DT_INT64, DT_FLOAT16, DT_BFLOAT16 = 2, 3, 5, 6, 9, 11

(OFX_OK, OFX_EINVAL, OFX_EDEVICE, OFX_ENOMEM, OFX_EUNSUPPORTED, OFX_ECOMM, OFX_EWORKSPACE, OFX_EPLAN,
 OFX_EINTERNAL) = range(9)
DEBUG_PLAN_SPIN_LIMIT, DEBUG_THROW_IN_COMPUTE, DEBUG_EXCHANGE_STALL = 1, 2, 3
REDUCE_SUM, REDUCE_MEAN, REDUCE_MAX, REDUCE_MIN = 0, 1, 2, 3
MEMCPY_H2D, MEMCPY_D2H, MEMCPY_D2D, MEMCPY_DEFAULT = 1, 2, 3, 4
UNIQUE_ID_BYTES = 128
PEER_HANDLE_BYTES = 96
PEER_MAX_RANKS = 16


class OfxError(RuntimeError):

    def __init__(self, code: int, msg: str):
        super().__init__(msg)
        self.code = code


STRUCT_MAGIC = 0x4F465831


class _Versioned(ctypes.Structure):

    def __init__(self, *args, **kw):
        super().__init__(ctypes.sizeof(type(self)), STRUCT_MAGIC, *args, **kw)


class Options(_Versioned):
    _fields_ = [("struct_size", ctypes.c_uint32), ("magic", ctypes.c_uint32),
                ("split_threshold", ctypes.c_int64), ("chunk", ctypes.c_int64),
                ("ordered", ctypes.c_int32), ("variant", ctypes.c_int32),
                ("heavy_threshold", ctypes.c_int64), ("planned", ctypes.c_int32),
                ("reserved", ctypes.c_int32), ("range_nnz", ctypes.c_int64)]


class SpmmAttrs(_Versioned):
    _fields_ = [("struct_size", ctypes.c_uint32), ("magic", ctypes.c_uint32),
# ... 132 lines not shown
        "ofx_edge_softmax_csr_heads_cpu": ([i32, i32, i32, i64, i64, i64, p, p, p, i64, i64, popt],
                                           i32),
        "ofx_edge_softmax_csr_heads_grad": ([p, i32, i32, i64, i64, i64, p, p, p, p, i64, i64, p,
                                             sz, popt], i32),
        "ofx_edge_softmax_csr_heads_grad_cpu": ([i32, i32, i32, i64, i64, i64, p, p, p, p, i64, i64,
                                                 popt], i32),
        "ofx_functional_edge_softmax_csr_heads": ([p, pdesc, pdesc, pdesc, pdesc, p, sz,
                                                   ctypes.POINTER(sz)], i32),
        "ofx_functional_edge_softmax_csr_heads_grad": ([p, pdesc, pdesc, pdesc, pdesc, pdesc, p, sz,
                                                        ctypes.POINTER(sz)], i32),
        "ofx_coo_to_csr_workspace_size": ([i32, i64, i64, i64, ctypes.POINTER(sz)], i32),
        "ofx_coo_to_csr": ([p, i32, i32, i64, i64, i64, p, p, p, i32, p, p, p, p, p, p, sz], i32),
        "ofx_coo_to_csr_cpu": ([i32, i32, i64, i64, i64, p, p, p, i32, p, p, p, ctypes.POINTER(i64)], i32),
        "ofx_balanced_range": ([i64, i64, i64, ctypes.POINTER(i64), ctypes.POINTER(i64)], i32),
        "ofx_csr_row_slice": ([p, i32, p, i64, i64, p], i32),
        "ofx_csr_row_slice_host": ([i32, p, i64, i64, p, ctypes.POINTER(i64), ctypes.POINTER(i64)], i32),
        "ofx_device_count": ([ctypes.POINTER(i32)], i32),
        "ofx_set_device": ([i32], i32),
        "ofx_get_device": ([ctypes.POINTER(i32)], i32),
        "ofx_device_synchronize": ([], i32),
        "ofx_malloc": ([ctypes.POINTER(p), sz], i32),
        "ofx_free": ([p], i32),
        "ofx_host_malloc": ([ctypes.POINTER(p), sz], i32),
        "ofx_host_free": ([p], i32),
        "ofx_stream_create": ([ctypes.POINTER(p)], i32),
        "ofx_stream_destroy": ([p], i32),
        "ofx_stream_sync": ([p], i32),
        "ofx_memcpy_async": ([p, p, p, sz, i32], i32),
        "ofx_memset_async": ([p, p, i32, sz], i32),
        "ofx_event_create": ([ctypes.POINTER(p), i32], i32),
        "ofx_event_destroy": ([p], i32),
        "ofx_event_record": ([p, p], i32),
        "ofx_event_sync": ([p], i32),
        "ofx_event_elapsed_ms": ([p, p, ctypes.POINTER(ctypes.c_float)], i32),
        "ofx_stream_wait_event": ([p, p], i32),
        "ofx_graph_exec_create": ([ctypes.POINTER(p)], i32),
        "ofx_graph_exec_destroy": ([p], i32),
        "ofx_graph_exec_stats": ([p, ctypes.POINTER(i32), ctypes.POINTER(i64), ctypes.POINTER(i64),
                                  ctypes.POINTER(i64)], i32),
        "ofx_stream_begin_capture": ([p], i32),
        "ofx_stream_is_capturing": ([p, ctypes.POINTER(i32)], i32),
        "ofx_stream_end_capture": ([p, p], i32),
        "ofx_graph_launch": ([p, p], i32),
        "ofx_comm_get_unique_id": ([p], i32),
        "ofx_comm_init_rank": ([ctypes.POINTER(p), i32, p, i32], i32),
        "ofx_comm_init_rank_deadline": ([ctypes.POINTER(p), i32, p, i32, ctypes.c_double], i32),
        "ofx_comm_set_timeouts": ([p, ctypes.c_double, ctypes.c_double], i32),
        "ofx_comm_abort": ([p], i32),
        "ofx_comm_destroy": ([p], i32),
        "ofx_comm_count": ([p, ctypes.POINTER(i32), ctypes.POINTER(i32)], i32),
        "ofx_allgather": ([p, p, p, sz, i32, p], i32),
        "ofx_allgather_p2p": ([p, p, sz, i32, p], i32),
        "ofx_peer_export": ([p, p], i32),
        "ofx_peer_open": ([p, ctypes.POINTER(p)], i32),
        "ofx_peer_close": ([p], i32),
        "ofx_peer_publish": ([p], i32),
        "ofx_peer_pull": ([p, i32, i32, p, p, u64], i32),
        "ofx_peer_pull_host": ([i32, i32, p, p, u64], i32),
        "ofx_allgather_pull": ([p, p, p, p, sz, i32], i32),
        "ofx_exchange_rows": ([p, p, i32, i64, p, p, p, p, p, p], i32),
        "ofx_spmm_rowsplit": ([p, p, i32, i32, i64, i64, i64, i64, p, p, p, p, p, i64, p, sz, popt], i32),
        "ofx_padded_owner_remap": ([p, i32, i64, i64, i64, p, p], i32),
        "ofx_gather_rows": ([p, i32, i64, i64, p, p, i64, p, i64], i32),
        "ofx_synth_row_ptr": ([i64, i64, i64, ctypes.c_double, u64, p], i32),
        "ofx_synth_columns": ([i64, i64, ctypes.c_double, u64, p, i64, i64, i32, p, i32], i32),
        "ofx_synth_values_host": ([i32, i64, i64, u64, i32, p], i32),
        "ofx_synth_dense": ([p, i32, i64, i64, i64, i64, u64, i32, p], i32),
        "ofx_synth_dense_host": ([i32, i64, i64, i64, i64, u64, i32, p], i32),
        "ofx_functional_spmm_csr_infer": ([pdesc, pdesc, pdesc, i64, i64, pdesc, pdesc], i32),
        "ofx_functional_spmm_csr_tmp_size": ([pdesc, pdesc, pdesc, i64, i64, pdesc,
                                              ctypes.POINTER(sz)], i32),
        "ofx_functional_spmm_csr": ([p, pdesc, pdesc, pdesc, i64, i64, pdesc, pdesc, p, sz], i32),
        "ofx_functional_spmm_csr_ex": ([p, pdesc, pdesc, pdesc, i64, i64, pdesc, pdesc, p, sz, i64,
                                        i64, i32, i32], i32),
        "ofx_functional_spmm_csr_global": ([p, pdesc, pdesc, pdesc, i64, i64, pdesc, i64, pdesc, p,
                                            sz, i32, ctypes.POINTER(i64), ctypes.POINTER(i32), i64,
                                            i32, ctypes.POINTER(sz)], i32),
        "ofx_functional_spmm_csr_global_attrs": ([p, pdesc, pdesc, pdesc, i64, i64, pdesc, i64, pdesc,
                                                  p, sz, i32, ctypes.POINTER(i64),
                                                  ctypes.POINTER(i32), i64, i32, ctypes.POINTER(sz),
                                                  pattrs], i32),
        "ofx_spmm_static_plans": ([ctypes.POINTER(i64), ctypes.POINTER(i64), ctypes.POINTER(i64),
                                   i32], i32),
        "ofx_functional_sddmm_csr": ([p, pdesc, pdesc, pdesc, pdesc, i64, i64, pdesc, p, sz,
                                      ctypes.POINTER(sz)], i32),
        "ofx_functional_sddmm_csr_attrs": ([p, pdesc, pdesc, pdesc, pdesc, i64, i64, pdesc, p, sz,
                                            ctypes.POINTER(sz), pattrs], i32),
        "ofx_functional_spmm_csr_gathered": ([p, pdesc, pdesc, pdesc, pdesc, pdesc, i64, i64, pdesc,
                                              p, sz, ctypes.POINTER(sz)], i32),
        "ofx_functional_spmm_csr_gathered_attrs": ([p, pdesc, pdesc, pdesc, pdesc, pdesc, i64, i64,
                                                    pdesc, p, sz, ctypes.POINTER(sz), pattrs], i32),
        "ofx_functional_csr_transpose": ([p, pdesc, pdesc, i64, i64, pdesc, pdesc, pdesc, p, sz,
                                          ctypes.POINTER(sz)], i32),
        "ofx_functional_spmm_csr_reduce": ([p, pdesc, pdesc, pdesc, i64, i64, pdesc, i32, pdesc,
                                            pdesc, p, sz, i64, i64, i32, i64, i32,
                                            ctypes.POINTER(sz)], i32),
        "ofx_functional_spmm_csr_reduce_grad_b": ([p, pdesc, pdesc, pdesc, pdesc, pdesc, pdesc, i64,
                                                   i64, pdesc, p, sz, ctypes.POINTER(sz)], i32),
        "ofx_functional_spmm_csr_reduce_grad_values": ([p, pdesc, pdesc, pdesc, pdesc, pdesc, i64,
                                                        i64, pdesc, p, sz, ctypes.POINTER(sz)],
                                                       i32),
        "ofx_op_spmm_csr_sbp_signatures": ([ctypes.c_char_p, sz], i32),
        "ofx_process_ctx_init": ([i64, i64, KV_PUSH_FN, KV_PULL_FN, SENDRECV_FN, p], i32),
        "ofx_ccl_registered": ([i32, ctypes.POINTER(i32), ctypes.POINTER(i32)], i32),
        "ofx_boxing_check_ccl_s2b": ([ppl, i32, ctypes.POINTER(i64), ctypes.c_char_p,
                                      ctypes.c_char_p], i32),
        "ofx_boxing_ccl_s2b": ([p, ppl, pdesc, pdesc, i64], i32),
        "ofx_nccl_logical_all_gather": ([p, ppl, pdesc, pdesc, ctypes.c_char_p], i32),
        "ofx_insert_nccl_logical_op": ([ctypes.c_char_p, ctypes.c_char_p, i32, ctypes.POINTER(i64),
                                        i64, p, sz], i32),
        "ofx_rccl_comm_key": ([ppl, ctypes.c_char_p, i64, i64, p, sz, ctypes.POINTER(i32)], i32),
        "ofx_spmm_job_create": ([ppl, i32, i32, i64, i64, i64, i64, ctypes.c_char_p,
                                 ctypes.POINTER(p)], i32),
        "ofx_spmm_job_describe": ([p, p, sz, ctypes.POINTER(sz)], i32),
        "ofx_spmm_job_run": ([p, p, p, p, p, p, p, p, sz], i32),
        "ofx_spmm_job_destroy": ([p], i32),
# ... 34 lines not shown
```

Baseline: 3725 GFLOP/s.

## Reuse SpMM plans across calls with device-side verification against row_ptr changes

Adds a plan-reuse table that keeps a built SpMM schedule and workspace across calls keyed on the CSR shape. Each row carries a claim check, so the compute kernel skips or falls back when row lengths no longer match. Stale flags and mismatch counts go through mapped host memory and events. It also adds a chunked walk routine that batches loads for hub rows. The aim is to drop repeated planning passes over row_ptr, at the cost of extra per-row checks, more workspace, and complex cache-invalidation logic.

```diff
diff --git a/include/ofx_spmm.h b/include/ofx_spmm.h
--- a/include/ofx_spmm.h
+++ b/include/ofx_spmm.h
@@ -33,6 +33,7 @@
 #define OFX_DEBUG_PLAN_SPIN_LIMIT 1
 #define OFX_DEBUG_THROW_IN_COMPUTE 2
 #define OFX_DEBUG_EXCHANGE_STALL 3
+#define OFX_DEBUG_OP_VARIANT 4
 int ofx_debug_set(int knob, int64_t value);
 
 #define OFX_STRUCT_MAGIC 0x4F465831u
@@ -73,6 +74,18 @@
 int ofx_spmm_csr_plan(void* stream, int idx_dtype, int val_dtype, int64_t m, int64_t k, int64_t n,
                       int64_t nnz, const void* row_ptr, int64_t row_begin, int64_t row_end,
                       void* workspace, size_t workspace_bytes, const ofx_spmm_options* opts);
+
+int ofx_spmm_csr_kept_workspace_size(int idx_dtype, int val_dtype, int64_t m, int64_t k, int64_t n,
+                                     int64_t nnz, int64_t row_begin, int64_t row_end,
+                                     const ofx_spmm_options* opts, size_t* bytes);
+int ofx_spmm_csr_plan_kept(void* stream, int idx_dtype, int val_dtype, int64_t m, int64_t k,
+                           int64_t n, int64_t nnz, const void* row_ptr, int64_t row_begin,
+                           int64_t row_end, void* workspace, size_t workspace_bytes,
+                           const ofx_spmm_options* opts, void* stale_word, uint64_t* host_counters);
+int ofx_spmm_csr_kept_mismatch_rows(void* stream, int idx_dtype, int val_dtype, int64_t m,
+                                    int64_t k, int64_t n, int64_t nnz, int64_t row_begin,
+                                    int64_t row_end, const void* workspace,
+                                    const ofx_spmm_options* opts, uint64_t* rows);
 
 int ofx_spmm_csr_describe(int idx_dtype, int val_dtype, int64_t m, int64_t k, int64_t n,
                           int64_t nnz, const void* b, int64_t ldb, const void* c, int64_t ldc,
@@ -290,6 +303,8 @@
 int ofx_event_destroy(void* event);
 int ofx_event_record(void* event, void* stream);
 int ofx_event_sync(void* event);
+int ofx_event_query(void* event, int* done);
+int ofx_host_malloc_mapped(void** host_ptr, void** device_ptr, size_t bytes);
 int ofx_event_elapsed_ms(void* start, void* end, float* ms);
 int ofx_stream_wait_event(void* stream, void* event);
 int ofx_graph_exec_create(void** exec);
@@ -401,6 +416,9 @@
     size_t tmp_bytes, int hierarchy_ndim, const int64_t* hierarchy, const int32_t* out_split_axes,
     int64_t parallel_id, int num_threads, size_t* tmp_size_out, const ofx_spmm_attrs* attrs);
 int ofx_spmm_static_plans(int64_t* entries, int64_t* plans, int64_t* hits, int release);
+int ofx_spmm_plan_reuse_set(int enable, int* previous);
+int ofx_spmm_plan_reuse_stats(int64_t* entries, int64_t* plans, int64_t* hits,
+                              int64_t* mismatch_rows, int64_t* stale, int64_t* dead);
 
 int ofx_functional_spmm_csr_ex(void* stream, const ofx_tensor_desc* row_ptr,
                                const ofx_tensor_desc* col_idx, const ofx_tensor_desc* values,
diff --git a/of-spmm_amd/csrc/device_shim.cpp b/of-spmm_amd/csrc/device_shim.cpp
--- a/of-spmm_amd/csrc/device_shim.cpp
+++ b/of-spmm_amd/csrc/device_shim.cpp
@@ -120,6 +120,23 @@
     return OFX_OK;
   });
 }
+extern "C" int ofx_host_malloc_mapped(void** host_ptr, void** device_ptr, size_t bytes) {
+  return ::ofx::guarded(__func__, [&]() -> int {
+    OFX_REQUIRE(host_ptr && device_ptr, OFX_EINVAL, "host_malloc_mapped: NULL");
+    *host_ptr = *device_ptr = nullptr;
+    void* p = nullptr;
+    OFX_HIP_CHECK(hipHostMalloc(&p, bytes ? bytes : 1, hipHostMallocMapped | hipHostMallocPortable));
+    void* d = nullptr;
+    if (hipHostGetDevicePointer(&d, p, 0) != hipSuccess || d == nullptr) {
+      (void)hipGetLastError();
+      d = p;
+    }
+    std::memset(p, 0, bytes ? bytes : 1);
+    *host_ptr = p;
+    *device_ptr = d;
+    return OFX_OK;
+  });
+}
 extern "C" int ofx_host_free(void* ptr) {
   return ::ofx::guarded(__func__, [&]() -> int {
     if (ptr) OFX_HIP_CHECK(hipHostFree(ptr));
@@ -195,6 +212,20 @@
   return ::ofx::guarded(__func__, [&]() -> int {
     OFX_HIP_CHECK(hipEventSynchronize(static_cast<hipEvent_t>(event)));
     OFX_TAKE_DEVICE_ERROR("event_sync");
+    return OFX_OK;
+  });
+}
+extern "C" int ofx_event_query(void* event, int* done) {
+  return ::ofx::guarded(__func__, [&]() -> int {
+    OFX_REQUIRE(done, OFX_EINVAL, "event_query: NULL");
+    const hipError_t e = hipEventQuery(static_cast<hipEvent_t>(event));
+    if (e == hipErrorNotReady) {
+      (void)hipGetLastError();
+      *done = 0;
+      return OFX_OK;
+    }
+    OFX_HIP_CHECK(e);
+    *done = 1;
     return OFX_OK;
   });
 }
diff --git a/of-spmm_amd/csrc/spmm_common.h b/of-spmm_amd/csrc/spmm_common.h
--- a/of-spmm_amd/csrc/spmm_common.h
+++ b/of-spmm_amd/csrc/spmm_common.h
@@ -145,6 +145,8 @@
   int32_t force_bin;
 };
 
+constexpr int32_t kPlannedVerified = 2;
+
 static inline Schedule resolve_schedule(int64_t n, const ofx_spmm_options* o) {
   Schedule s;
   s.variant = o ? o->variant : 0;
diff --git a/of-spmm_amd/csrc/spmm_csr.hip b/of-spmm_amd/csrc/spmm_csr.hip
--- a/of-spmm_amd/csrc/spmm_csr.hip
+++ b/of-spmm_amd/csrc/spmm_csr.hip
@@ -188,11 +188,12 @@
   });
 }
 
-extern "C" int ofx_spmm_csr_plan(void* stream, int idx_dtype, int val_dtype, int64_t m,
-                                 int64_t k, int64_t n, int64_t nnz, const void* row_ptr,
-                                 int64_t row_begin, int64_t row_end, void* workspace,
-                                 size_t workspace_bytes, const ofx_spmm_options* opts) {
-  return ::ofx::guarded(__func__, [&]() -> int {
+namespace ofx {
+namespace {
+int plan_entry(void* stream, int idx_dtype, int val_dtype, int64_t m, int64_t k, int64_t n,
+               int64_t nnz, const void* row_ptr, int64_t row_begin, int64_t row_end,
+               void* workspace, size_t workspace_bytes, const ofx_spmm_options* opts, int kept,
+               void* stale_word, uint64_t* host_counters) {
     OFX_TAKE_DEVICE_ERROR("spmm_csr_plan");
     OFX_READ_OPTIONS(opts, "spmm_csr_plan");
     int rc = check_common(idx_dtype, val_dtype, m, k, n, nnz);
@@ -208,9 +209,12 @@
     const plan::WsLayout w = plan::ws_layout(nrows, nnz, n, acc_bytes_of(val_dtype), s);
     if (w.total == 0) return OFX_OK;
     OFX_REQUIRE(row_ptr != nullptr, OFX_EINVAL, "spmm_csr_plan: NULL row_ptr");
-    OFX_REQUIRE(workspace != nullptr && workspace_bytes >= w.total, OFX_EWORKSPACE,
+    const size_t ws_need = kept ? plan::verified_total(w, nrows) : w.total;
+    OFX_REQUIRE(workspace != nullptr && workspace_bytes >= ws_need, OFX_EWORKSPACE,
                 "spmm_csr_plan: workspace of %zu bytes is smaller than the %zu bytes required",
-                workspace_bytes, w.total);
+                workspace_bytes, ws_need);
+    OFX_REQUIRE(!kept || nnz <= (int64_t)UINT32_MAX, OFX_EINVAL,
+                "spmm_csr_plan_kept: nnz=%lld does not fit the verify block", (long long)nnz);
     hipStream_t st = static_cast<hipStream_t>(stream);
   #ifdef OFX_DEBUG_BOUNDS
     {
@@ -222,11 +226,89 @@
   #endif
     plan::WorkList wl{};
     char* ws = static_cast<char*>(workspace);
+    unsigned* claimed = kept ? plan::claimed_of(w, ws) : nullptr;
     if (idx_dtype == OFX_DT_INT32)
-      return plan::launch_plan<int32_t>(st, static_cast<const int32_t*>(row_ptr), row_begin, nrows,
-                                        nnz_est, s, w, ws, &wl);
-    return plan::launch_plan<int64_t>(st, static_cast<const int64_t*>(row_ptr), row_begin, nrows,
-                                      nnz_est, s, w, ws, &wl);
+      rc = plan::launch_plan<int32_t>(st, static_cast<const int32_t*>(row_ptr), row_begin, nrows,
+                                      nnz_est, s, w, ws, &wl, claimed,
+                                      static_cast<unsigned*>(stale_word));
+    else
+      rc = plan::launch_plan<int64_t>(st, static_cast<const int64_t*>(row_ptr), row_begin, nrows,
+                                      nnz_est, s, w, ws, &wl, claimed,
+                                      static_cast<unsigned*>(stale_word));
+    if (rc == OFX_OK && host_counters != nullptr)
+      OFX_HIP_CHECK(hipMemcpyAsync(host_counters, wl.counters, 4 * sizeof(uint64_t),
+                                   hipMemcpyDeviceToHost, st));
+    return rc;
+}
+}
+}
+
+extern "C" int ofx_spmm_csr_plan(void* stream, int idx_dtype, int val_dtype, int64_t m,
+                                 int64_t k, int64_t n, int64_t nnz, const void* row_ptr,
+                                 int64_t row_begin, int64_t row_end, void* workspace,
+                                 size_t workspace_bytes, const ofx_spmm_options* opts) {
+  return ::ofx::guarded(__func__, [&]() -> int {
+    return plan_entry(stream, idx_dtype, val_dtype, m, k, n, nnz, row_ptr, row_begin, row_end,
+                      workspace, workspace_bytes, opts, 0, nullptr, nullptr);
+  });
+}
+
+extern "C" int ofx_spmm_csr_kept_workspace_size(int idx_dtype, int val_dtype, int64_t m, int64_t k,
+                                                int64_t n, int64_t nnz, int64_t row_begin,
+                                                int64_t row_end, const ofx_spmm_options* opts,
+                                                size_t* bytes) {
+  return ::ofx::guarded(__func__, [&]() -> int {
+    OFX_REQUIRE(bytes != nullptr, OFX_EINVAL, "spmm_csr_kept_workspace_size: bytes is NULL");
+    *bytes = 0;
+    OFX_READ_OPTIONS(opts, "spmm_csr_kept_workspace_size");
+    int rc = check_common(idx_dtype, val_dtype, m, k, n, nnz);
+    if (rc) return rc;
+    OFX_REQUIRE(0 <= row_begin && row_begin <= row_end && row_end <= m, OFX_EINVAL,
+                "spmm_csr_kept_workspace_size: row range [%lld, %lld) outside [0, %lld)",
+                (long long)row_begin, (long long)row_end, (long long)m);
+    const int64_t nrows = row_end - row_begin;
+    if (nrows == 0 || n == 0 || nnz > (int64_t)UINT32_MAX) return OFX_OK;
+    const int64_t nnz_est = launch_nnz(m, nrows, nnz, opts);
+    const Schedule s = launch_schedule(nrows, nnz_est, n, resolve_schedule(n, opts));
+    if (use_small_form(nrows, nnz_est, n, s)) return OFX_OK;
+    const plan::WsLayout w = plan::ws_layout(nrows, nnz, n, acc_bytes_of(val_dtype), s);
+    if (w.total > 0) *bytes = plan::verified_total(w, nrows);
+    return OFX_OK;
+  });
+}
+
+extern "C" int ofx_spmm_csr_plan_kept(void* stream, int idx_dtype, int val_dtype, int64_t m,
+                                      int64_t k, int64_t n, int64_t nnz, const void* row_ptr,
+                                      int64_t row_begin, int64_t row_end, void* workspace,
+                                      size_t workspace_bytes, const ofx_spmm_options* opts,
+                                      void* stale_word, uint64_t* host_counters) {
+  return ::ofx::guarded(__func__, [&]() -> int {
+    return plan_entry(stream, idx_dtype, val_dtype, m, k, n, nnz, row_ptr, row_begin, row_end,
+                      workspace, workspace_bytes, opts, 1, stale_word, host_counters);
+  });
+}
+
+extern "C" int ofx_spmm_csr_kept_mismatch_rows(void* stream, int idx_dtype, int val_dtype,
+                                               int64_t m, int64_t k, int64_t n, int64_t nnz,
+                                               int64_t row_begin, int64_t row_end,
+                                               const void* workspace, const ofx_spmm_options* opts,
+                                               uint64_t* rows) {
+  return ::ofx::guarded(__func__, [&]() -> int {
+    OFX_REQUIRE(rows != nullptr && workspace != nullptr, OFX_EINVAL,
+                "spmm_csr_kept_mismatch_rows: NULL argument");
+    OFX_READ_OPTIONS(opts, "spmm_csr_kept_mismatch_rows");
+    const int64_t nrows = row_end - row_begin;
+    const int64_t nnz_est = launch_nnz(m, nrows, nnz, opts);
+    const Schedule s = launch_schedule(nrows, nnz_est, n, resolve_schedule(n, opts));
+    const plan::WsLayout w = plan::ws_layout(nrows, nnz, n, acc_bytes_of(val_dtype), s);
+    OFX_REQUIRE(w.total > 0, OFX_EINVAL, "spmm_csr_kept_mismatch_rows: this launch has no plan");
+    const char* hdr = static_cast<const char*>(workspace) + plan::verify_offset(w);
+    hipStream_t st = static_cast<hipStream_t>(stream);
+    unsigned long long v = 0;
+    OFX_HIP_CHECK(hipMemcpyAsync(&v, hdr, sizeof(v), hipMemcpyDeviceToHost, st));
+    OFX_HIP_CHECK(hipStreamSynchronize(st));
+    *rows = v;
+    return OFX_OK;
   });
 }
 
diff --git a/of-spmm_amd/csrc/spmm_csr_impl.h b/of-spmm_amd/csrc/spmm_csr_impl.h
--- a/of-spmm_amd/csrc/spmm_csr_impl.h
+++ b/of-spmm_amd/csrc/spmm_csr_impl.h
@@ -535,6 +535,76 @@
     __builtin_nontemporal_store(__builtin_bit_cast(R, o), reinterpret_cast<R*>(p));
   } else {
     *reinterpret_cast<Pack<T, VEC>*>(p) = o;
+  }
+}
+
+#ifndef OFX_WALK_LOADS
+#define OFX_WALK_LOADS 4
+#endif
+template <typename T, typename I, typename K>
+__device__ __forceinline__ void accumulate_walk(const I* __restrict__ col, const T* __restrict__ val,
+                                                const I* __restrict__ vperm,
+                                                const BRows<T, K::BUF>& br, int64_t j0, int64_t j1,
+                                                bool active,
+                                                typename Num<T>::acc (&acc)[K::VEC]) {
+#pragma clang fp contract(off)
+  constexpr int VEC = K::VEC, kWalk = OFX_WALK_LOADS;
+  using A = typename Num<T>::acc;
+  using P = Pack<T, VEC>;
+  for (int64_t j = j0; j < j1; j += kWalk) {
+    const int cnt = (int)((j1 - j) < kWalk ? (j1 - j) : kWalk);
+    P bv[kWalk];
+    A vv[kWalk];
+#pragma unroll
+    for (int u = 0; u < kWalk; ++u) {
+      vv[u] = A(0);
+      if (u < cnt) {
+        const I cu = OFX_LD(col + (j + u));
+        const int64_t jv = vperm ? (int64_t)OFX_LD(vperm + (j + u)) : j + u;
+        vv[u] = Num<T>::load(OFX_LD(val + jv));
+        if (active) bv[u] = br.template load<false, P>(cu);
+      }
+    }
+#pragma unroll
+    for (int u = 0; u < kWalk; ++u) {
+      if (u < cnt && active) {
+#pragma unroll
+        for (int e = 0; e < VEC; ++e) acc[e] = acc[e] + Num<T>::mul(vv[u], Num<T>::load(bv[u].v[e]));
+      }
+    }
+  }
+}
+
+template <typename T, typename I, typename K>
+__device__ __forceinline__ void walk_hub_row(const I* __restrict__ col, const T* __restrict__ val,
+                                             const I* __restrict__ vperm, const T* __restrict__ B,
+                                             int64_t ldb, int64_t kb, T* __restrict__ crow, int64_t n,
+                                             int64_t rs, int64_t re, int64_t chunk, int gl,
+                                             const T* __restrict__ bias, int act) {
+#pragma clang fp contract(off)
+  constexpr int VEC = K::VEC, LPR = K::LPR;
+  using A = typename Num<T>::acc;
+  const int64_t nck = num_chunks(re - rs, chunk);
+  for (int64_t c0 = 0; c0 < n; c0 += (int64_t)LPR * VEC) {
+    int64_t cc = c0 + (int64_t)gl * VEC;
+    const bool active = cc < n;
+    if constexpr (K::SH) {
+      if (active && cc + VEC > n) cc = n - VEC;
+    }
+    const BRows<T, K::BUF> br = brows<T, K::BUF>(B, c0, cc, active, ldb, kb);
+    A acc[VEC];
+#pragma unroll
+    for (int e = 0; e < VEC; ++e) acc[e] = A(0);
+    for (int64_t q = 0; q < nck; ++q) {
+      A pa[VEC];
+#pragma unroll
+      for (int e = 0; e < VEC; ++e) pa[e] = A(0);
+      const int64_t a0 = rs + q * chunk;
+      accumulate_walk<T, I, K>(col, val, vperm, br, a0, q == nck - 1 ? re : a0 + chunk, active, pa);
+#pragma unroll
+      for (int e = 0; e < VEC; ++e) acc[e] = acc[e] + pa[e];
+    }
+    if (active) store_row<T, VEC, false>(crow + cc, acc, bias ? bias + cc : nullptr, act);
   }
 }
 
@@ -928,7 +998,8 @@
                      const int64_t* __restrict__ items, const int64_t* __restrict__ order,
                      typename Num<T>::acc* __restrict__ part, const T* __restrict__ bias,
                      int act, int64_t wave_blocks, int64_t block_base,
-                     unsigned* __restrict__ arrive, unsigned* err) {
+                     unsigned* __restrict__ arrive, unsigned* err,
+                     const unsigned* __restrict__ claimed) {
   using A = typename Num<T>::acc;
   constexpr int VEC = K::VEC, LPR = K::LPR, kWaves = K::WPB;
   const int64_t bid = block_base + (int64_t)blockIdx.x;
@@ -962,6 +1033,7 @@
         wc = uniform64(wc);
         const int64_t rs = (int64_t)OFX_LD(rp + (row_begin + wr));
         const int64_t re = (int64_t)OFX_LD(rp + (row_begin + wr + 1));
+        if (claimed != nullptr && !plan::claim_holds(claimed, wr, re - rs)) continue;
         int64_t j0 = rs, j1 = re;
         if (wc >= 0) {
           j0 = rs + wc * chunk;
@@ -1019,6 +1091,7 @@
       wc = uniform64(wc);
       const int64_t rs = (int64_t)OFX_LD(rp + (row_begin + wr));
       const int64_t re = (int64_t)OFX_LD(rp + (row_begin + wr + 1));
+      if (claimed != nullptr && !plan::claim_holds(claimed, wr, re - rs)) return;
       int64_t j0 = rs, j1 = re;
       if (wc >= 0) {
         j0 = rs + wc * chunk;
@@ -1062,8 +1135,9 @@
 #else
   constexpr bool kIdx = true;
 #endif
+  constexpr int64_t kWalkRow = -2;
   int64_t lr, c = -1;
-  bool by_index = false;
+  bool by_index = false, item = false;
   if (order == nullptr) {
     if (g >= nrows) return;
     lr = g;
@@ -1079,9 +1153,11 @@
     if (g < nchunks) {
       lr = OFX_LD(items + (2 * g + 0));
       c = OFX_LD(items + (2 * g + 1));
+      item = true;
     } else if (g < nchunks + nheavy || !idx) {
       const int64_t q = g - nchunks;
       if (q >= nrows - nhubs) return;
+      item = g < nchunks + nheavy;
       lr = plan::order_row(order, nrows, nheavy, q);
     } else {
       lr = g - nchunks - nheavy;
@@ -1095,8 +1171,14 @@
   }
   const int64_t rs = (int64_t)OFX_LD(rp + (row_begin + lr));
   const int64_t re = (int64_t)OFX_LD(rp + (row_begin + lr + 1));
-  if (by_index && (re - rs > split || re - rs > heavy)) return;
-  int64_t j0 = rs, j1 = re;
+  if (by_index && (re - rs > split || re - rs > heavy)) {
+    if (claimed == nullptr || plan::claim_holds(claimed, lr, re - rs)) return;
+    if (gl == 0) plan::note_mismatch(claimed);
+    if (re - rs > split) c = kWalkRow;
+  } else if (claimed != nullptr && item) {
+    if (!plan::claim_holds(claimed, lr, re - rs)) return;
+  }
+  int64_t j0 = rs, j1 = c == kWalkRow ? rs : re;
   if (c >= 0) {
     j0 = rs + c * chunk;
     j1 = (re - j0 - chunk < chunk) ? re : j0 + chunk;
@@ -1115,7 +1197,7 @@
     if (active) {
       if (c >= 0)
         store_partial<A, VEC, K::LR>(part + g * n + cc, acc);
-      else
+      else if (c == -1)
         store_row<T, VEC, K::NT>(C + lr * ldc + cc, acc, bias ? bias + cc : nullptr, act);
     }
   }
@@ -1124,15 +1206,22 @@
       hub_tail<T, VEC, LPR, K::SH>(arrive, g - c, num_chunks(re - rs, chunk), part, C, ldc, lr, n,
                                    gl, true, gbase, bias, act);
   }
-}
-
-
-template <typename T, int VEC, int L>
+  if (c == kWalkRow) {
+    const int64_t ws_ = (int64_t)OFX_LD(rp + (row_begin + lr));
+    const int64_t we_ = (int64_t)OFX_LD(rp + (row_begin + lr + 1));
+    walk_hub_row<T, I, K>(col, val, vperm, B, ldb, kb, C + lr * ldc, n, ws_, we_, chunk, gl, bias, act);
+  }
+}
+
+
+template <typename T, typename I, int VEC, int L>
 __global__ void __launch_bounds__(kBlock)
     spmm_reduce_kernel(const unsigned long long* __restrict__ counters,
                        const int64_t* __restrict__ hubs,
                        const typename Num<T>::acc* __restrict__ part, T* __restrict__ C,
-                       int64_t ldc, int64_t n, const T* __restrict__ bias, int act) {
+                       int64_t ldc, int64_t n, const T* __restrict__ bias, int act,
+                       const I* __restrict__ rp, int64_t row_begin,
+                       const unsigned* __restrict__ claimed) {
 #pragma clang fp contract(off)
   using A = typename Num<T>::acc;
   using P = Pack<A, VEC>;
@@ -1145,6 +1234,10 @@
     const int64_t lr = OFX_LD(hubs + (3 * h + 0));
     const int64_t slot = OFX_LD(hubs + (3 * h + 1));
     const int64_t nc = OFX_LD(hubs + (3 * h + 2));
+    if (claimed != nullptr) {
+      const int64_t len = (int64_t)OFX_LD(rp + (row_begin + lr + 1)) - (int64_t)OFX_LD(rp + (row_begin + lr));
+      if (!plan::claim_holds(claimed, lr, len)) continue;
+    }
     for (int64_t c = (int64_t)gl * VEC; c < n; c += (int64_t)L * VEC) {
       const A* p = part + slot * n + c;
       A acc[VEC];
@@ -1173,10 +1266,11 @@
   }
 }
 
-template <typename T, int VEC>
+template <typename T, typename I, int VEC>
 int launch_reduce_vec(hipStream_t s, int64_t max_hubs, int64_t n,
                       const unsigned long long* counters, const int64_t* hubs,
-                      const typename Num<T>::acc* part, T* C, int64_t ldc, const T* bias, int act) {
+                      const typename Num<T>::acc* part, T* C, int64_t ldc, const T* bias, int act,
+                      const I* rp, int64_t row_begin, const unsigned* claimed) {
   const int64_t lanes = (n + VEC - 1) / VEC;
   int l = 4;
   while (l < 64 && l < lanes) l *= 2;
@@ -1184,8 +1278,8 @@
   int64_t grid = (max_hubs + per_block - 1) / per_block;
   if (grid > kMaxReduceBlocks) grid = kMaxReduceBlocks;
 #define OFX_REDUCE(LL)                                                                        \
-  hipLaunchKernelGGL((spmm_reduce_kernel<T, VEC, LL>), dim3((unsigned)grid), dim3(kBlock), 0, s, \
-                     counters, hubs, part, C, ldc, n, bias, act)
+  hipLaunchKernelGGL((spmm_reduce_kernel<T, I, VEC, LL>), dim3((unsigned)grid), dim3(kBlock), 0, s, \
+                     counters, hubs, part, C, ldc, n, bias, act, rp, row_begin, claimed)
   switch (l) {
     case 4: OFX_REDUCE(4); break;
     case 8: OFX_REDUCE(8); break;
@@ -1198,15 +1292,17 @@
   return OFX_OK;
 }
 
-template <typename T>
+template <typename T, typename I>
 int launch_reduce(hipStream_t s, int64_t max_hubs, int64_t n, const unsigned long long* counters,
                   const int64_t* hubs, const typename Num<T>::acc* part, T* C, int64_t ldc,
-                  const T* bias, int act) {
+                  const T* bias, int act, const I* rp, int64_t row_begin, const unsigned* claimed) {
   using A = typename Num<T>::acc;
   constexpr int kVec = 16 / (int)sizeof(A);
   if ((n * (int64_t)sizeof(A)) % 16 == 0)
-    return launch_reduce_vec<T, kVec>(s, max_hubs, n, counters, hubs, part, C, ldc, bias, act);
-  return launch_reduce_vec<T, 1>(s, max_hubs, n, counters, hubs, part, C, ldc, bias, act);
+    return launch_reduce_vec<T, I, kVec>(s, max_hubs, n, counters, hubs, part, C, ldc, bias, act, rp,
+                                         row_begin, claimed);
+  return launch_reduce_vec<T, I, 1>(s, max_hubs, n, counters, hubs, part, C, ldc, bias, act, rp,
+                                    row_begin, claimed);
 }
 
 int pick_vec(int elem_bytes, const Launch& L, int forced_vec, int cap = 16) {
@@ -1294,10 +1390,14 @@
   if (const int rc = debug_publish<T, I, K>(L, 1)) return rc;
 #endif
   WorkList wl{};
+  const bool verified = plan && L.sched.planned == kPlannedVerified;
+  const unsigned* claimed = nullptr;
   if (plan) {
-    OFX_REQUIRE(L.ws != nullptr && L.ws_bytes >= w.total, OFX_EWORKSPACE,
+    const size_t ws_need = verified ? plan::verified_total(w, L.nrows) : w.total;
+    OFX_REQUIRE(L.ws != nullptr && L.ws_bytes >= ws_need, OFX_EWORKSPACE,
                 "spmm_csr: workspace of %zu bytes is smaller than the %zu bytes required",
-                L.ws_bytes, w.total);
+                L.ws_bytes, ws_need);
+    if (verified) claimed = plan::claimed_of(w, static_cast<char*>(L.ws));
     if (L.sched.planned) {
       plan::worklist_of(w, static_cast<char*>(L.ws), &wl);
     } else {
@@ -1328,12 +1428,12 @@
                        C, L.ldc, L.row_begin, L.nrows, L.n, plan ? L.sched.split : INT64_MAX,
                        plan ? L.sched.chunk : INT64_MAX, heavy, counters, items, order, part,
                        static_cast<const T*>(L.bias), L.act, wave_blocks, b0, wl.arrive,
-                       plan ? device_error_words() : nullptr);
+                       plan ? device_error_words() : nullptr, claimed);
     OFX_HIP_CHECK(hipGetLastError());
   }
   if (plan && w.max_hubs > 0 && !K::LR)
-    return launch_reduce<T>(L.stream, w.max_hubs, L.n, counters, hub, part, C, L.ldc,
-                            static_cast<const T*>(L.bias), L.act);
+    return launch_reduce<T, I>(L.stream, w.max_hubs, L.n, counters, hub, part, C, L.ldc,
+                               static_cast<const T*>(L.bias), L.act, rp, L.row_begin, claimed);
   return OFX_OK;
 }
 
diff --git a/of-spmm_amd/csrc/spmm_plan.h b/of-spmm_amd/csrc/spmm_plan.h
--- a/of-spmm_amd/csrc/spmm_plan.h
+++ b/of-spmm_amd/csrc/spmm_plan.h
@@ -67,6 +67,27 @@
 __device__ __forceinline__ void raise_device_error(unsigned* err, int which) {
   if (err != nullptr)
     __hip_atomic_store(err + which, 1u, __ATOMIC_RELAXED, __HIP_MEMORY_SCOPE_SYSTEM);
+}
+
+struct VerifyHdr {
+  unsigned long long mismatch_rows;
+  unsigned* stale;
+};
+constexpr size_t kVerifyHdrBytes = 256;
+__host__ __device__ __forceinline__ VerifyHdr* verify_hdr(const unsigned* claimed) {
+  return reinterpret_cast<VerifyHdr*>(
+      reinterpret_cast<char*>(const_cast<unsigned*>(claimed)) - kVerifyHdrBytes);
+}
+__device__ __forceinline__ bool claim_holds(const unsigned* __restrict__ claimed, int64_t lr,
+                                            int64_t len) {
+  return (int64_t)OFX_LDP(claimed + lr) == len;
+}
+__device__ __forceinline__ void note_mismatch(const unsigned* claimed) {
+  VerifyHdr* h = verify_hdr(claimed);
+  if (!OFX_DOK(h, sizeof(VerifyHdr))) return;
+  __hip_atomic_fetch_add(&h->mismatch_rows, 1ull, __ATOMIC_RELAXED, __HIP_MEMORY_SCOPE_AGENT);
+  unsigned* st = h->stale;
+  if (st != nullptr) __hip_atomic_store(st, 1u, __ATOMIC_RELAXED, __HIP_MEMORY_SCOPE_SYSTEM);
 }
 
 template <typename I>
@@ -218,7 +239,8 @@
                      unsigned long long host_tag, int64_t nblocks,
                      unsigned long long* __restrict__ counters, int64_t* __restrict__ hubs,
                      int64_t* __restrict__ items, int64_t* __restrict__ order,
-                     unsigned* __restrict__ arrive, int spin_limit, unsigned* err) {
+                     unsigned* __restrict__ arrive, int spin_limit, unsigned* err,
+                     unsigned* __restrict__ claimed, unsigned* stale) {
   __shared__ int64_t s_off[kPlanVals];
   __shared__ int s_fail;
   int cls[RPT];
@@ -329,6 +351,20 @@
 #pragma unroll
   for (int i = 0; i < kPlanVals; ++i) off[i] = s_off[i];
   plan_write_rows(cls, nc, v, off, base, nrows, hubs, items, order, arrive);
+  if (claimed != nullptr) {
+#pragma unroll
+    for (int q = 0; q < RPT; ++q) {
+      const int64_t g = base + q;
+      if (g >= nrows) continue;
+      const bool listed = cls[q] == -1 || (cls[q] == 0 && kBins > 1);
+      unsigned len = 0;
+      if (listed)
+        len = (unsigned)((int64_t)OFX_LDP(rp + (row_begin + g + 1)) -
+                         (int64_t)OFX_LDP(rp + (row_begin + g)));
+      OFX_STP(claimed + g, len);
+    }
+    if (b == 0 && threadIdx.x == 0) OFX_STP(&verify_hdr(claimed)->stale, stale);
+  }
 }
 
 struct WsLayout {
@@ -392,9 +428,18 @@
   return (splitmix64(counter.fetch_add(1)) >> 2) | 1ull;
 }
 
+inline size_t verify_offset(const WsLayout& w) { return align_up(w.total, 256); }
+inline size_t verified_total(const WsLayout& w, int64_t nrows) {
+  return verify_offset(w) + kVerifyHdrBytes + align_up((size_t)nrows * sizeof(unsigned), 256);
+}
+inline unsigned* claimed_of(const WsLayout& w, char* ws) {
+  return reinterpret_cast<unsigned*>(ws + verify_offset(w) + kVerifyHdrBytes);
+}
+
 template <typename I>
 int launch_plan(hipStream_t stream, const I* rp, int64_t row_begin, int64_t nrows, int64_t nnz,
-                const Schedule& sched, const WsLayout& w, char* ws, WorkList* wl) {
+                const Schedule& sched, const WsLayout& w, char* ws, WorkList* wl,
+                unsigned* claimed = nullptr, unsigned* stale = nullptr) {
   const int64_t heavy = sched.heavy == 0 ? auto_heavy(nrows, nnz) : sched.heavy;
   worklist_of(w, ws, wl);
   auto* look = reinterpret_cast<unsigned long long*>(ws + w.look);
@@ -406,12 +451,12 @@
     hipLaunchKernelGGL((spmm_plan_kernel<4, I>), dim3((unsigned)w.plan_blocks), dim3(kBlock), 0,
                        stream, rp, row_begin, nrows, sched.split, sched.chunk, heavy, look, host_tag,
                        w.plan_blocks, wl->counters, wl->hubs, wl->items, wl->order, wl->arrive,
-                       spin, err);
+                       spin, err, claimed, stale);
   else
     hipLaunchKernelGGL((spmm_plan_kernel<16, I>), dim3((unsigned)w.plan_blocks), dim3(kBlock), 0,
                        stream, rp, row_begin, nrows, sched.split, sched.chunk, heavy, look, host_tag,
                        w.plan_blocks, wl->counters, wl->hubs, wl->items, wl->order, wl->arrive,
-                       spin, err);
+                       spin, err, claimed, stale);
   OFX_HIP_CHECK(hipGetLastError());
   return OFX_OK;
 }
diff --git a/of-spmm_amd/oneflow/core/framework/framework.cpp b/of-spmm_amd/oneflow/core/framework/framework.cpp
--- a/of-spmm_amd/oneflow/core/framework/framework.cpp
+++ b/of-spmm_amd/oneflow/core/framework/framework.cpp
@@ -17,6 +17,8 @@
     default: break;
   }
 }
+
+int TestHookVariant() { return (int)ofx::debug_knob(OFX_DEBUG_OP_VARIANT, 0); }
 
 const char* DataType_Name(DataType dt) {
   switch (dt) {
diff --git a/of-spmm_amd/oneflow/core/framework/framework.h b/of-spmm_amd/oneflow/core/framework/framework.h
--- a/of-spmm_amd/oneflow/core/framework/framework.h
+++ b/of-spmm_amd/oneflow/core/framework/framework.h
@@ -154,6 +154,7 @@
   } while (0)
 
 void TestHookCompute(const char* op_name);
+int TestHookVariant();
 
 template <typename T>
 struct GetDataType;
diff --git a/of-spmm_amd/oneflow/core/functional/spmm_functor.cpp b/of-spmm_amd/oneflow/core/functional/spmm_functor.cpp
--- a/of-spmm_amd/oneflow/core/functional/spmm_functor.cpp
+++ b/of-spmm_amd/oneflow/core/functional/spmm_functor.cpp
@@ -2,6 +2,7 @@
 
 #include "oneflow/core/framework/framework.h"
 #include "oneflow/core/functional/spmm_functor.h"
+#include "oneflow/user/kernels/spmm_plan_state.h"
 #include "ofx_internal.h"
 #include "ofx_spmm.h"
 
@@ -226,7 +227,7 @@
       *state = kernel->CreateOpKernelState(&ictx);
     }
     kstate = state->get();
-  } else if (static_csr != 0) {
+  } else if (static_csr != 0 || dev == DeviceType::kHIP) {
     kstate = EagerKernelState(reg, kernel, b->device, dev);
   }
   user_op::KernelCacheContext cache_ctx(ParallelContext(pl.parallel_id, pl.parallel_num()),
@@ -348,6 +349,31 @@
     if (entries) *entries = e;
     if (plans) *plans = p;
     if (hits) *hits = h;
+    return OFX_OK;
+  });
+}
+
+extern "C" int ofx_spmm_plan_reuse_set(int enable, int* previous) {
+  return ::ofx::guarded(__func__, [&]() -> int {
+    const int prev = PlanReuseSwitch().exchange(enable != 0 ? 1 : 0);
+    if (previous) *previous = prev;
+    return OFX_OK;
+  });
+}
+
+extern "C" int ofx_spmm_plan_reuse_stats(int64_t* entries, int64_t* plans, int64_t* hits,
+                                         int64_t* mismatch_rows, int64_t* stale, int64_t* dead) {
+  return ::ofx::guarded(__func__, [&]() -> int {
+    PlanReuseStats s;
+    std::lock_guard<std::mutex> lock(g_eager_states_mu);
+    for (auto& kv : g_eager_states)
+      if (kv.second) SpmmCsrPlanReuseStats(kv.second.get(), &s);
+    if (entries) *entries = s.entries;
+    if (plans) *plans = s.plans;
+    if (hits) *hits = s.hits;
+    if (mismatch_rows) *mismatch_rows = s.mismatch_rows;
+    if (stale) *stale = s.stale;
+    if (dead) *dead = s.dead;
     return OFX_OK;
   });
 }
@@ -531,7 +557,8 @@
   std::shared_ptr<user_op::OpKernelCache> cache;
   auto sc = attrs.find("static_csr");
   user_op::OpKernelState* kstate = nullptr;
-  if (sc != attrs.end() && static_cast<int64_t>(sc->second) != 0)
+  if ((sc != attrs.end() && static_cast<int64_t>(sc->second) != 0) ||
+      (rc.device_type() == DeviceType::kHIP && std::string(op_name) == "fused_spmm_csr"))
     kstate = EagerKernelState(reg, kernel, device, rc.device_type());
   try {
     if (pl != nullptr) {
diff --git a/of-spmm_amd/oneflow/core/functional/spmm_functor.h b/of-spmm_amd/oneflow/core/functional/spmm_functor.h
--- a/of-spmm_amd/oneflow/core/functional/spmm_functor.h
+++ b/of-spmm_amd/oneflow/core/functional/spmm_functor.h
@@ -18,6 +18,8 @@
 
 bool SpmmCsrPlanStateStats(user_op::OpKernelState* state, int64_t* entries, int64_t* plans,
                            int64_t* hits, bool release);
+struct PlanReuseStats;
+bool SpmmCsrPlanReuseStats(user_op::OpKernelState* state, PlanReuseStats* sum);
 
 int EdgeSoftmaxCsr(void* stream, const ofx_tensor_desc* row_ptr, const ofx_tensor_desc* col_idx,
                    const ofx_tensor_desc* in, const ofx_tensor_desc* grad, ofx_tensor_desc* out,
diff --git a/of-spmm_amd/oneflow/user/kernels/spmm_kernel.cpp b/of-spmm_amd/oneflow/user/kernels/spmm_kernel.cpp
--- a/of-spmm_amd/oneflow/user/kernels/spmm_kernel.cpp
+++ b/of-spmm_amd/oneflow/user/kernels/spmm_kernel.cpp
@@ -4,6 +4,19 @@
 #include "ofx_spmm.h"
 
 namespace oneflow {
+
+bool SpmmCsrPlanReuseStats(user_op::OpKernelState* state, PlanReuseStats* sum) {
+  auto* s = dynamic_cast<SpmmCsrPlanState*>(state);
+  if (s == nullptr) return false;
+  const PlanReuseStats r = s->ReuseStats();
+  sum->entries += r.entries;
+  sum->dead += r.dead;
+  sum->plans += r.plans;
+  sum->hits += r.hits;
+  sum->stale += r.stale;
+  sum->mismatch_rows += r.mismatch_rows;
+  return true;
+}
 
 bool SpmmCsrPlanStateStats(user_op::OpKernelState* state, int64_t* entries, int64_t* plans,
                            int64_t* hits, bool release) {
@@ -49,6 +62,7 @@
 ofx_spmm_options OptionsOf(const SpmmCsrOpKernelCache* cache) {
   ofx_spmm_options o = OFX_SPMM_OPTIONS_INIT;
   if (cache != nullptr) o.split_threshold = ofx_spmm_default_split(cache->logical_n());
+  o.variant = TestHookVariant();
   return o;
 }
 
@@ -67,13 +81,51 @@
   const SpmmCsrPlanState::Key key{static_csr, row_ptr, plans->key_on_stream() ? stream : nullptr,
                                   hs->device_index(), idx_dt, val_dt, m, k, n, nnz, row_begin,
                                   row_end, opts->split_threshold, opts->chunk,
-                                  opts->heavy_threshold, opts->range_nnz};
+                                  opts->heavy_threshold, opts->range_nnz, opts->variant};
   auto plan = [&](void* sws, size_t bytes) {
     return ofx_spmm_csr_plan(stream, idx_dt, val_dt, m, k, n, nnz, row_ptr, row_begin, row_end,
                              sws, bytes, opts);
   };
   if (UseStaticPlan(plans, key, need, hs->IsGraphCapturing(), op_name, plan, ws, ws_bytes, sp))
     opts->planned = 1;
+}
+
+void UseReusedSpmmPlan(SpmmCsrPlanState* plans, ep::HipStream* hs, const void* row_ptr, int idx_dt,
+                       int val_dt, int64_t m, int64_t k, int64_t n, int64_t nnz, int64_t row_begin,
+                       int64_t row_end, const char* op_name, ofx_spmm_options* opts, void** ws,
+                       size_t* ws_bytes, StaticPlan* sp) {
+  if (row_end <= row_begin || n <= 0 || PlanReuseSwitch().load(std::memory_order_relaxed) == 0)
+    return;
+  size_t need = 0;
+  if (ofx_spmm_csr_kept_workspace_size(idx_dt, val_dt, m, k, n, nnz, row_begin, row_end, opts,
+                                       &need) != OFX_OK || need == 0)
+    return;
+  void* stream = hs->hip_stream();
+  const bool capturing = hs->IsGraphCapturing();
+  sp->hold = std::unique_lock<std::recursive_mutex>(plans->launch_mutex());
+  sp->key = SpmmCsrPlanState::Key{0, row_ptr, plans->key_on_stream() ? stream : nullptr,
+                                  hs->device_index(), idx_dt, val_dt, m, k, n, nnz, row_begin,
+                                  row_end, opts->split_threshold, opts->chunk,
+                                  opts->heavy_threshold, opts->range_nnz, opts->variant};
+  const PlanReuseDecision d = plans->reuse().OnCall(sp->key, need, capturing, stream);
+  if (d.action == PlanReuseAction::kPlain) {
+    sp->hold.unlock();
+    return;
+  }
+  sp->keyed = true;
+  if (d.action == PlanReuseAction::kPlanKept) {
+    const int rc = ofx_spmm_csr_plan_kept(stream, idx_dt, val_dt, m, k, n, nnz, row_ptr, row_begin,
+                                          row_end, d.ws, d.bytes, opts, d.stale_dev,
+                                          d.host_counters);
+    if (rc != OFX_OK) plans->reuse().Fail(sp->key, stream, capturing);
+    OFX_KERNEL_CHECK(rc == OFX_OK, op_name << " kernel failed (" << rc << "): " << ofx_last_error());
+    plans->reuse().Planned(sp->key, stream);
+    opts->planned = 1;
+  } else {
+    opts->planned = 2;
+  }
+  *ws = d.ws;
+  *ws_bytes = d.bytes;
 }
 
 template <DeviceType device_type>
@@ -123,11 +175,17 @@
     if (plans != nullptr && static_csr != 0)
       UseStaticSpmmPlan(plans, static_csr, hs, row_ptr->dptr(), idx_dt, val_dt, m, k, n, nnz,
                         row_begin, row_end, op_name, &opts, &ws, &ws_bytes, &sp);
+    else if (plans != nullptr)
+      UseReusedSpmmPlan(plans, hs, row_ptr->dptr(), idx_dt, val_dt, m, k, n, nnz, row_begin,
+                        row_end, op_name, &opts, &ws, &ws_bytes, &sp);
     rc = ofx_spmm_csr_fused(stream, idx_dt, val_dt, m, k, n, nnz, row_ptr->dptr(),
                             col_idx->dptr(), values->dptr(), b->dptr(), b->row_stride(),
                             out->mut_dptr(), out->row_stride(), row_begin, row_end, bias_ptr, act,
                             ws, ws_bytes, &opts);
-    if (rc != OFX_OK && sp.keyed) plans->Drop(sp.key, hs->IsGraphCapturing());
+    if (rc != OFX_OK && sp.keyed) {
+      if (static_csr != 0) plans->Drop(sp.key, hs->IsGraphCapturing());
+      else plans->reuse().Fail(sp.key, stream, hs->IsGraphCapturing());
+    }
   } else {
     const int threads = ctx->stream()->As<ep::CpuStream>()->num_threads();
     rc = ofx_spmm_csr_fused_cpu(threads, idx_dt, val_dt, m, k, n, nnz, row_ptr->dptr(),
@@ -287,6 +345,7 @@
   const user_op::TensorDesc* out_logical = ctx->LogicalTensorDesc4ArgNameAndIndex("out", 0);
   ofx_spmm_options o = OFX_SPMM_OPTIONS_INIT;
   if (out_logical != nullptr) o.split_threshold = ofx_spmm_default_split(out_logical->shape().At(1));
+  o.variant = TestHookVariant();
   size_t bytes = 0;
   const int rc = ofx_spmm_csr_workspace_size(
       DtCode(row_ptr.data_type()), DtCode(b.data_type()), ctx->Attr<int64_t>("a_num_rows"),
diff --git a/of-spmm_amd/oneflow/user/kernels/spmm_plan_reuse.h b/of-spmm_amd/oneflow/user/kernels/spmm_plan_reuse.h
--- /dev/null
+++ b/of-spmm_amd/oneflow/user/kernels/spmm_plan_reuse.h
@@ -0,0 +1,256 @@
+#ifndef OFX_ONEFLOW_USER_KERNELS_SPMM_PLAN_REUSE_H_
+#define OFX_ONEFLOW_USER_KERNELS_SPMM_PLAN_REUSE_H_
+
+#include <stddef.h>
+#include <stdint.h>
+
+#include <list>
+#include <vector>
+
+namespace oneflow {
+
+struct SpmmPlanKey {
+  int64_t static_csr;
+  const void* row_ptr;
+  const void* stream;
+  int device, idx_dt, val_dt;
+  int64_t m, k, n, nnz, row_begin, row_end, split, chunk, heavy, range_nnz;
+  int64_t variant = 0;
+  bool operator==(const SpmmPlanKey& o) const {
+    return static_csr == o.static_csr && row_ptr == o.row_ptr && stream == o.stream &&
+           device == o.device && idx_dt == o.idx_dt && val_dt == o.val_dt && m == o.m &&
+           k == o.k && n == o.n && nnz == o.nnz && row_begin == o.row_begin &&
+           row_end == o.row_end && split == o.split && chunk == o.chunk && heavy == o.heavy &&
+           range_nnz == o.range_nnz && variant == o.variant;
+  }
+};
+
+struct PlanReuseHostBlock {
+  uint64_t counters[4];
+  volatile unsigned stale;
+};
+
+enum class PlanReuseAction {
+  kPlain,
+  kPlanKept,
+  kReuse,
+};
+
+struct PlanReuseDecision {
+  PlanReuseAction action = PlanReuseAction::kPlain;
+  void* ws = nullptr;
+  size_t bytes = 0;
+  void* stale_dev = nullptr;
+  uint64_t* host_counters = nullptr;
+};
+
+struct PlanReuseStats {
+  int64_t entries = 0;
+  int64_t dead = 0;
+  int64_t plans = 0;
+  int64_t hits = 0;
+  int64_t stale = 0;
+  int64_t mismatch_rows = 0;
+};
+
+template <typename Dev>
+class PlanReuseTable {
+ public:
+  static constexpr size_t kMaxEntries = 8;
+  static constexpr size_t kSeenKeys = 32;
+  static constexpr int kMaxStales = 2;
+  static constexpr int64_t kIdxExcluded = 16;
+
+  explicit PlanReuseTable(Dev dev = Dev()) : dev_(dev) {}
+  ~PlanReuseTable() { Release(); }
+  PlanReuseTable(const PlanReuseTable&) = delete;
+  PlanReuseTable& operator=(const PlanReuseTable&) = delete;
+
+  PlanReuseDecision OnCall(const SpmmPlanKey& key, size_t kept_bytes, bool capturing,
+                           void* stream) {
+    PlanReuseDecision d;
+    if (kept_bytes == 0) return d;
+    for (auto it = entries_.begin(); it != entries_.end(); ++it) {
+      if (!(it->key == key)) continue;
+      entries_.splice(entries_.begin(), entries_, it);
+      Entry& e = entries_.front();
+      if (e.state == State::kDead || e.bytes < kept_bytes) return d;
+      if (e.state == State::kPlanning) {
+        if (capturing || !dev_.EventDone(e.ready)) return d;
+        const int64_t nhubs = (int64_t)e.host->counters[1];
+        const int64_t nheavy = (int64_t)e.host->counters[3] - (int64_t)e.host->counters[2];
+        if ((nhubs + nheavy) * kIdxExcluded > key.row_end - key.row_begin) {
+          Kill(&e, stream, true);
+          return d;
+        }
+        e.state = State::kReusable;
+      }
+      if (e.host->stale != 0 && !e.pinned && !capturing) {
+        ++stale_;
+        e.host->stale = 0;
+        if (++e.stales >= kMaxStales) {
+          Kill(&e, stream, true);
+          return d;
+        }
+        e.state = State::kPlanning;
+        ++plans_;
+        return Fill(e, PlanReuseAction::kPlanKept, stream);
+      }
+      if (capturing) e.pinned = true;
+      ++hits_;
+      return Fill(e, PlanReuseAction::kReuse, stream);
+    }
+    if (capturing) return d;
+    if (!Seen(key)) return d;
+    if (entries_.size() >= kMaxEntries) Evict(stream);
+    Entry e;
+    e.key = key;
+    e.bytes = kept_bytes;
+    if (dev_.Malloc(key.device, &e.ws, kept_bytes) != 0) return d;
+    if (dev_.Zero(stream, e.ws, kept_bytes) != 0 || dev_.HostAlloc(&e.host, &e.stale_dev) != 0 ||
+        dev_.EventCreate(&e.ready) != 0) {
+      Destroy(&e);
+      return d;
+    }
+    e.host->stale = 0;
+    for (uint64_t& c : e.host->counters) c = 0;
+    entries_.push_front(e);
+    ++plans_;
+    return Fill(entries_.front(), PlanReuseAction::kPlanKept, stream);
+  }
+
+  void Planned(const SpmmPlanKey& key, void* stream) {
+    if (Entry* e = Find(key)) {
+      if (dev_.EventRecord(e->ready, stream) != 0) Kill(e, stream, false);
+    }
+  }
+
+  void Fail(const SpmmPlanKey& key, void* stream, bool capturing) {
+    if (Entry* e = Find(key)) Kill(e, stream, !capturing);
+  }
+
+  PlanReuseStats Stats() {
+    PlanReuseStats s;
+    s.plans = plans_;
+    s.hits = hits_;
+    s.stale = stale_;
+    s.mismatch_rows = mismatch_freed_;
+    for (Entry& e : entries_) {
+      if (e.state == State::kDead) ++s.dead; else ++s.entries;
+      if (e.ws != nullptr) s.mismatch_rows += (int64_t)dev_.MismatchRows(e.key, e.ws, e.last_stream);
+    }
+    for (Entry& e : retired_) s.mismatch_rows += (int64_t)dev_.MismatchRows(e.key, e.ws, e.last_stream);
+    return s;
+  }
+
+  void Release() {
+    for (auto* list : {&retired_, &entries_}) {
+      for (Entry& e : *list) {
+        if (e.ws != nullptr) {
+          dev_.Drain(e.key.device);
+          mismatch_freed_ += (int64_t)dev_.MismatchRows(e.key, e.ws, nullptr);
+        }
+        Destroy(&e);
+      }
+      list->clear();
+    }
+    seen_.clear();
+    seen_next_ = 0;
+  }
+
+ private:
+  enum class State { kPlanning, kReusable, kDead };
+  struct Entry {
+    SpmmPlanKey key{};
+    void* ws = nullptr;
+    size_t bytes = 0;
+    PlanReuseHostBlock* host = nullptr;
+    void* stale_dev = nullptr;
+    void* ready = nullptr;
+    void* last_stream = nullptr;
+    State state = State::kPlanning;
+    bool pinned = false;
+    int stales = 0;
+  };
+
+  PlanReuseDecision Fill(Entry& e, PlanReuseAction a, void* stream) {
+    e.last_stream = stream;
+    PlanReuseDecision d;
+    d.action = a;
+    d.ws = e.ws;
+    d.bytes = e.bytes;
+    d.stale_dev = e.stale_dev;
+    d.host_counters = e.host->counters;
+    return d;
+  }
+
+  Entry* Find(const SpmmPlanKey& key) {
+    for (Entry& e : entries_)
+      if (e.key == key) return &e;
+    return nullptr;
+  }
+
+  bool Seen(const SpmmPlanKey& key) {
+    for (const SpmmPlanKey& k : seen_)
+      if (k == key) return true;
+    if (seen_.size() < kSeenKeys) {
+      seen_.push_back(key);
+    } else {
+      seen_[seen_next_] = key;
+      seen_next_ = (seen_next_ + 1) % kSeenKeys;
+    }
+    return false;
+  }
+
+  void Kill(Entry* e, void* stream, bool can_wait) {
+    e->state = State::kDead;
+    RetireWorkspace(e, stream, can_wait);
+  }
+
+  void RetireWorkspace(Entry* e, void* stream, bool can_wait) {
+    if (e->ws == nullptr) return;
+    if (can_wait && !e->pinned && (e->last_stream == stream || e->last_stream == nullptr) &&
+        dev_.EventRecord(e->ready, stream) == 0 && dev_.EventSync(e->ready) == 0) {
+      mismatch_freed_ += (int64_t)dev_.MismatchRows(e->key, e->ws, stream);
+      dev_.Free(e->key.device, e->ws);
+    } else {
+      Entry r;
+      r.key = e->key;
+      r.ws = e->ws;
+      r.bytes = e->bytes;
+      r.last_stream = nullptr;
+      retired_.push_back(r);
+    }
+    e->ws = nullptr;
+  }
+
+  void Evict(void* stream) {
+    auto victim = entries_.end();
+    for (auto it = entries_.begin(); it != entries_.end(); ++it)
+      if (!it->pinned) victim = it;
+    if (victim == entries_.end()) return;
+    RetireWorkspace(&*victim, stream, true);
+    Destroy(&*victim);
+    entries_.erase(victim);
+  }
+
+  void Destroy(Entry* e) {
+    if (e->ws != nullptr) dev_.Free(e->key.device, e->ws);
+    if (e->host != nullptr) dev_.HostFree(e->host);
+    if (e->ready != nullptr) dev_.EventDestroy(e->ready);
+    e->ws = nullptr;
+    e->host = nullptr;
+    e->ready = nullptr;
+  }
+
+  Dev dev_;
+  std::list<Entry> entries_;
+  std::list<Entry> retired_;
+  std::vector<SpmmPlanKey> seen_;
+  size_t seen_next_ = 0;
+  int64_t plans_ = 0, hits_ = 0, stale_ = 0, mismatch_freed_ = 0;
+};
+
+}
+
+#endif
diff --git a/of-spmm_amd/oneflow/user/kernels/spmm_plan_state.h b/of-spmm_amd/oneflow/user/kernels/spmm_plan_state.h
--- a/of-spmm_amd/oneflow/user/kernels/spmm_plan_state.h
+++ b/of-spmm_amd/oneflow/user/kernels/spmm_plan_state.h
@@ -1,31 +1,87 @@
 #ifndef OFX_ONEFLOW_USER_KERNELS_SPMM_PLAN_STATE_H_
 #define OFX_ONEFLOW_USER_KERNELS_SPMM_PLAN_STATE_H_
 
+#include <atomic>
+#include <cstdlib>
 #include <list>
 #include <mutex>
 
 #include "oneflow/core/framework/framework.h"
+#include "oneflow/user/kernels/spmm_plan_reuse.h"
 #include "ofx_spmm.h"
 
 namespace oneflow {
+
+struct HipPlanReuseDev {
+  template <typename F>
+  static int WithDevice(int device, F&& f) {
+    int prev = -1;
+    if (ofx_get_device(&prev) != OFX_OK) prev = -1;
+    if (prev != device && ofx_set_device(device) != OFX_OK) return OFX_EDEVICE;
+    const int rc = f();
+    if (prev >= 0 && prev != device) ofx_set_device(prev);
+    return rc;
+  }
+  int Malloc(int device, void** p, size_t bytes) {
+    return WithDevice(device, [&]() { return ofx_malloc(p, bytes); });
+  }
+  int Zero(void* stream, void* p, size_t bytes) { return ofx_memset_async(stream, p, 0, bytes); }
+  int Free(int device, void* p) {
+    return WithDevice(device, [&]() { return ofx_free(p); });
+  }
+  int HostAlloc(PlanReuseHostBlock** host, void** stale_dev) {
+    void *h = nullptr, *d = nullptr;
+    const int rc = ofx_host_malloc_mapped(&h, &d, sizeof(PlanReuseHostBlock));
+    if (rc != OFX_OK) return rc;
+    *host = static_cast<PlanReuseHostBlock*>(h);
+    *stale_dev = static_cast<char*>(d) + offsetof(PlanReuseHostBlock, stale);
+    return OFX_OK;
+  }
+  void HostFree(PlanReuseHostBlock* host) { ofx_host_free(host); }
+  int EventCreate(void** ev) { return ofx_event_create(ev, 0); }
+  void EventDestroy(void* ev) { ofx_event_destroy(ev); }
+  int EventRecord(void* ev, void* stream) { return ofx_event_record(ev, stream); }
+  bool EventDone(void* ev) {
+    int done = 0;
+    return ofx_event_query(ev, &done) == OFX_OK && done != 0;
+  }
+  int EventSync(void* ev) { return ofx_event_sync(ev); }
+  uint64_t MismatchRows(const SpmmPlanKey& key, const void* ws, void* stream) {
+    ofx_spmm_options o = OFX_SPMM_OPTIONS_INIT;
+    o.split_threshold = key.split;
+    o.chunk = key.chunk;
+    o.heavy_threshold = key.heavy;
+    o.range_nnz = key.range_nnz;
+    o.variant = (int32_t)key.variant;
+    uint64_t rows = 0;
+    WithDevice(key.device, [&]() {
+      return ofx_spmm_csr_kept_mismatch_rows(stream, key.idx_dt, key.val_dt, key.m, key.k, key.n,
+                                             key.nnz, key.row_begin, key.row_end, ws, &o, &rows);
+    });
+    return rows;
+  }
+  void Drain(int device) {
+    WithDevice(device, [&]() { return ofx_device_synchronize(); });
+  }
+};
+
+inline std::atomic<int>& PlanReuseSwitch() {
+  static std::atomic<int> on{[] {
+    const char* e = std::getenv("OFX_SPMM_PLAN_REUSE");
+    return (e != nullptr && e[0] == '0' && e[1] == 0) ? 0 : 1;
+  }()};
+  return on;
+}
 
 class SpmmCsrPlanState final : public user_op::OpKernelState {
  public:
-  struct Key {
-    int64_t static_csr;
-    const void* row_ptr;
-    const void* stream;
-    int device, idx_dt, val_dt;
-    int64_t m, k, n, nnz, row_begin, row_end, split, chunk, heavy, range_nnz;
-    bool operator==(const Key& o) const {
-      return static_csr == o.static_csr && row_ptr == o.row_ptr && stream == o.stream &&
-             device == o.device && idx_dt == o.idx_dt && val_dt == o.val_dt && m == o.m &&
-             k == o.k && n == o.n && nnz == o.nnz && row_begin == o.row_begin &&
-             row_end == o.row_end && split == o.split && chunk == o.chunk && heavy == o.heavy &&
-             range_nnz == o.range_nnz;
-    }
-  };
+  using Key = SpmmPlanKey;
   static constexpr size_t kMaxPlans = 8;
+  PlanReuseTable<HipPlanReuseDev>& reuse() { return reuse_; }
+  PlanReuseStats ReuseStats() {
+    std::lock_guard<std::recursive_mutex> lock(mu_);
+    return reuse_.Stats();
+  }
 
   explicit SpmmCsrPlanState(bool key_on_stream) : key_on_stream_(key_on_stream) {}
   ~SpmmCsrPlanState() override { Release(); }
@@ -97,6 +153,7 @@
 
   void Release() {
     std::lock_guard<std::recursive_mutex> lock(mu_);
+    reuse_.Release();
     for (auto* list : {&retired_, &entries_}) {
       for (Entry& e : *list) {
         WithDevice(e.key.device, [&]() {
@@ -130,6 +187,7 @@
   std::list<Entry> entries_;
   std::list<Entry> retired_;
   int64_t plans_ = 0, hits_ = 0;
+  PlanReuseTable<HipPlanReuseDev> reuse_;
 };
 
 struct StaticPlan {
diff --git a/of-spmm_amd/oneflow_spmm/_C.py b/of-spmm_amd/oneflow_spmm/_C.py
--- a/of-spmm_amd/oneflow_spmm/_C.py
+++ b/of-spmm_amd/oneflow_spmm/_C.py
@@ -147,6 +147,19 @@
     return {"entries": e.value, "plans": p.value, "hits": h.value}
 
 
+def plan_reuse_stats() -> dict:
+    vals = [ctypes.c_int64() for _ in range(6)]
+    check(LIB.ofx_spmm_plan_reuse_stats(*[ctypes.byref(v) for v in vals]), "spmm_plan_reuse_stats")
+    names = ("entries", "plans", "hits", "mismatch_rows", "stale", "dead")
+    return {k: v.value for k, v in zip(names, vals)}
+
+
+def plan_reuse(enable: bool) -> bool:
+    prev = ctypes.c_int()
+    check(LIB.ofx_spmm_plan_reuse_set(1 if enable else 0, ctypes.byref(prev)), "spmm_plan_reuse_set")
+    return bool(prev.value)
+
+
 def fused_spmm_csr(a_csr_row_ptr: torch.Tensor, a_csr_col_idx: torch.Tensor,
                    a_csr_values: torch.Tensor, a_num_rows: int, a_num_cols: int, b: torch.Tensor,
                    bias: torch.Tensor | None = None, *, relu: bool = False,
diff --git a/of-spmm_amd/oneflow_spmm/_lib.py b/of-spmm_amd/oneflow_spmm/_lib.py
--- a/of-spmm_amd/oneflow_spmm/_lib.py
+++ b/of-spmm_amd/oneflow_spmm/_lib.py
@@ -10,7 +10,7 @@
 
 (OFX_OK, OFX_EINVAL, OFX_EDEVICE, OFX_ENOMEM, OFX_EUNSUPPORTED, OFX_ECOMM, OFX_EWORKSPACE, OFX_EPLAN,
  OFX_EINTERNAL) = range(9)
-DEBUG_PLAN_SPIN_LIMIT, DEBUG_THROW_IN_COMPUTE, DEBUG_EXCHANGE_STALL = 1, 2, 3
+DEBUG_PLAN_SPIN_LIMIT, DEBUG_THROW_IN_COMPUTE, DEBUG_EXCHANGE_STALL, DEBUG_OP_VARIANT = 1, 2, 3, 4
 REDUCE_SUM, REDUCE_MEAN, REDUCE_MAX, REDUCE_MIN = 0, 1, 2, 3
 MEMCPY_H2D, MEMCPY_D2H, MEMCPY_D2D, MEMCPY_DEFAULT = 1, 2, 3, 4
 UNIQUE_ID_BYTES = 128
@@ -209,6 +209,8 @@
         "ofx_event_destroy": ([p], i32),
         "ofx_event_record": ([p, p], i32),
         "ofx_event_sync": ([p], i32),
+        "ofx_event_query": ([p, ctypes.POINTER(i32)], i32),
+        "ofx_host_malloc_mapped": ([ctypes.POINTER(p), ctypes.POINTER(p), sz], i32),
         "ofx_event_elapsed_ms": ([p, p, ctypes.POINTER(ctypes.c_float)], i32),
         "ofx_stream_wait_event": ([p, p], i32),
         "ofx_graph_exec_create": ([ctypes.POINTER(p)], i32),
@@ -259,6 +261,14 @@
                                                   pattrs], i32),
         "ofx_spmm_static_plans": ([ctypes.POINTER(i64), ctypes.POINTER(i64), ctypes.POINTER(i64),
                                    i32], i32),
+        "ofx_spmm_plan_reuse_set": ([i32, ctypes.POINTER(i32)], i32),
+        "ofx_spmm_plan_reuse_stats": ([ctypes.POINTER(i64)] * 6, i32),
+        "ofx_spmm_csr_kept_workspace_size": ([i32, i32, i64, i64, i64, i64, i64, i64, popt,
+                                              ctypes.POINTER(sz)], i32),
+        "ofx_spmm_csr_plan_kept": ([p, i32, i32, i64, i64, i64, i64, p, i64, i64, p, sz, popt, p,
+                                    p], i32),
+        "ofx_spmm_csr_kept_mismatch_rows": ([p, i32, i32, i64, i64, i64, i64, i64, i64, p, popt,
+                                             ctypes.POINTER(u64)], i32),
         "ofx_functional_sddmm_csr": ([p, pdesc, pdesc, pdesc, pdesc, i64, i64, pdesc, p, sz,
                                       ctypes.POINTER(sz)], i32),
         "ofx_functional_sddmm_csr_attrs": ([p, pdesc, pdesc, pdesc, pdesc, i64, i64, pdesc, p, sz,
```

Result: no change. 3716 GFLOP/s (-0.2%).
